# zhoujoey/ORB-SLAM3-Mac

Measured on AMD Instinct MI355X. Metric: ORB extract+match frames/sec, higher is better.
Workload: dtype u8; 1 GPU; vga: synthetic 640x480 batch=1024 per GPU, 8-level pyramid, 1000 feats/frame, ORB extract + Hamming 2-NN match (Frame.cc:1146) + SearchForInitialization (ORBmatcher.cc:710) vs successor frame; pipelines=1, matchers=side by side (two contexts), frames_total=1024

## Files before the change

include/orbhip.h:

```cpp
#ifndef ORBHIP_H
#define ORBHIP_H
#include <stddef.h>
#include <stdint.h>
#ifdef __cplusplus
extern "C" {
#endif

#define ORBHIP_OK 0
#define ORBHIP_E_BADARG (-1)
#define ORBHIP_E_NODEVICE (-2)
#define ORBHIP_E_HIP (-3)
#define ORBHIP_E_CAPACITY (-4)
#define ORBHIP_E_ABORTED (-5)
#define ORBHIP_E_NOTSPD (-6)
#define ORBHIP_E_EMPTY (-7)

typedef struct {
    float x, y, size, angle, response;
    int32_t octave, class_id;
} orbhip_keypoint;

typedef struct orbhip_ctx orbhip_ctx;
typedef struct orbhip_extractor orbhip_extractor;

const char *orbhip_version(void);
const char *orbhip_last_error(void);

int orbhip_ctx_create(int device, void *stream, orbhip_ctx **out);
void orbhip_ctx_destroy(orbhip_ctx *ctx);
int orbhip_ctx_synchronize(orbhip_ctx *ctx);
int orbhip_ctx_wait_for(orbhip_ctx *ctx, orbhip_ctx *other);
int orbhip_ctx_check_status(orbhip_ctx *ctx);
void *orbhip_ctx_stream(orbhip_ctx *ctx);

int orbhip_extractor_create(orbhip_ctx *ctx, int nfeatures, float scale_factor, int nlevels,
                            int ini_th_fast, int min_th_fast, orbhip_extractor **out);
void orbhip_extractor_destroy(orbhip_extractor *ext);

int orbhip_extractor_levels(const orbhip_extractor *ext);
int orbhip_extractor_table(const orbhip_extractor *ext, int which, float *out);
int orbhip_extractor_features_per_level(const orbhip_extractor *ext, int *out);
int orbhip_extractor_umax(const orbhip_extractor *ext, int *out16);

int orbhip_extractor_reserve(orbhip_extractor *ext, int width, int height, int max_batch);
int orbhip_extractor_max_keypoints(const orbhip_extractor *ext);

int orbhip_extract_batch_device(orbhip_extractor *ext, const uint8_t *d_images, int width,
                                int height, size_t row_stride, size_t frame_stride, int batch,
                                int lap0, int lap1);
int orbhip_extractor_results(orbhip_extractor *ext, orbhip_keypoint **d_kp, uint8_t **d_desc,
                             int32_t **d_count, int32_t **d_mono_index);
int orbhip_extract_batch_host(orbhip_extractor *ext, const uint8_t *h_images, int width, int height,
                              size_t row_stride, size_t frame_stride, int batch, int lap0, int lap1,
                              orbhip_keypoint *kp_out, uint8_t *desc_out, int cap,
                              int32_t *count_out, int32_t *mono_out);
int orbhip_extract_batch_host_view(orbhip_extractor *ext, const uint8_t *h_images, int width, int height, size_t row_stride,
                                   size_t frame_stride, int batch, int lap0, int lap1, const orbhip_keypoint **kp_view,
                                   const uint8_t **desc_view, int *row_capacity, const int32_t **count_view, const int32_t **mono_view);
int orbhip_extractor_blur_kernel(const orbhip_extractor *ext, int batch);

int orbhip_extractor_resize_band_rows(const orbhip_extractor *ext, int level);

int orbhip_extractor_last_frame(orbhip_extractor *ext, int frame, const orbhip_keypoint **d_kp, const uint8_t **d_desc,
                                const orbhip_keypoint **h_kp_view, const uint8_t **h_desc_view, int32_t *count, unsigned long long *generation);

int orbhip_extractor_level_dims(const orbhip_extractor *ext, int level, int *w, int *h);
int orbhip_extractor_get_pyramid_level(orbhip_extractor *ext, int frame, int level, int padded,
                                       uint8_t *h_out, size_t out_stride);
int orbhip_extractor_get_pyramid_padded(orbhip_extractor *ext, int frame, uint8_t *const *levels_out, const size_t *strides);
int orbhip_extractor_get_blurred_level(orbhip_extractor *ext, int frame, int level,
                                       uint8_t *h_out, size_t out_stride);
int orbhip_extractor_get_fast_candidates(orbhip_extractor *ext, int frame, int level,
                                         int32_t *xs, int32_t *ys, int32_t *scores, int cap,
                                         int32_t *n_out);
int orbhip_extractor_get_level_keypoints(orbhip_extractor *ext, int frame, int level,
                                         orbhip_keypoint *out, int cap, int32_t *n_out);

int orbhip_extractor_set_graph_mode(orbhip_extractor *ext, int enable);

#define ORBHIP_STAGE_PYRAMID 0
#define ORBHIP_STAGE_FAST_CELLS 1
#define ORBHIP_STAGE_BLUR 2
#define ORBHIP_STAGE_OCTREE 3
#define ORBHIP_STAGE_DESC 4
#define ORBHIP_STAGE_ASSEMBLE 5
#define ORBHIP_STAGE_COUNT 6
int orbhip_extractor_set_profiling(orbhip_extractor *ext, int enable);
int orbhip_extractor_stage_ms(orbhip_extractor *ext, float *ms_out );

int orbhip_descriptor_distance(const uint8_t *a32, const uint8_t *b32);

int orbhip_match_bf2nn_device(orbhip_ctx *ctx, const uint8_t *d_descA, const int32_t *d_nA,
                              size_t strideA, const uint8_t *d_descB, const int32_t *d_nB,
                              size_t strideB, int pairs, int max_n, double ratio,
                              int32_t *d_idx2, int32_t *d_dist2, uint8_t *d_accept);

int orbhip_search_for_initialization_device(orbhip_ctx *ctx,
        const orbhip_keypoint *d_kpA, const uint8_t *d_descA, const int32_t *d_nA,
        const orbhip_keypoint *d_kpB, const uint8_t *d_descB, const int32_t *d_nB,
        int pairs, int max_n, size_t frame_stride_kp , float min_x, float min_y,
        float max_x, float max_y, int window_size, float nn_ratio, int check_orientation,
        float *d_prev_matched, int32_t *d_matches12, int32_t *d_nmatches);

int orbhip_prev_matched_init_device(orbhip_ctx *ctx, const orbhip_keypoint *d_kp, size_t frame_stride_kp,
                                    int frames, int max_n, float *d_prev_matched);

typedef struct orbhip_proj_query {
    float u, v, radius, ur, angle;
    int32_t min_level, max_level, has_obs;
} orbhip_proj_query;
int orbhip_search_by_projection_device(orbhip_ctx *ctx, const orbhip_proj_query *d_q, const uint8_t *d_desc_q,
                                       const int32_t *d_nq, int max_q, const orbhip_keypoint *d_kp,
                                       const uint8_t *d_desc, const float *d_u_right, const int32_t *d_n, int max_n,
                                       size_t frame_stride_kp, int pairs, float min_x, float min_y, float max_x,
                                       float max_y, int th_high, int check_orientation, int32_t *d_train_match,
                                       int32_t *d_nmatches);

int orbhip_search_local_map_device(orbhip_ctx *ctx, const orbhip_proj_query *d_q, const uint8_t *d_desc_q,
                                   const int32_t *d_nq, int max_q, const orbhip_keypoint *d_kp,
                                   const uint8_t *d_desc, const float *d_u_right, const int32_t *d_n, int max_n,
                                   size_t frame_stride_kp, int pairs, float min_x, float min_y, float max_x,
                                   float max_y, int th_high, float nn_ratio, int32_t *d_train_match,
                                   int32_t *d_nmatches);

int orbhip_search_by_projection_rig_device(orbhip_ctx *ctx, int mode, const orbhip_proj_query *d_q, const uint8_t *d_desc_q,
                                           const int32_t *d_nq, int max_q, const orbhip_keypoint *d_kp, const uint8_t *d_desc,
                                           const int32_t *d_n, const int32_t *d_nleft, const int32_t *d_mirror, int max_n,
                                           size_t frame_stride_kp, int pairs, float min_x, float min_y, float max_x, float max_y,
                                           int th_high, float nn_ratio, int check_orientation, int32_t *d_train_match,
                                           int32_t *d_nmatches);

int orbhip_search_by_projection_host(orbhip_ctx *ctx, int mode, const orbhip_proj_query *q, const uint8_t *desc_q, int nq,
                                     const orbhip_keypoint *kp, const uint8_t *desc, const float *u_right, int n,
                                     float min_x, float min_y, float max_x, float max_y, int th_high, float nn_ratio,
                                     int check_orientation, int32_t *train_match_inout, int32_t *nmatches_out);
int orbhip_search_by_projection_rig_host(orbhip_ctx *ctx, int mode, const orbhip_proj_query *q, const uint8_t *desc_q, int nq,
                                         const orbhip_keypoint *kp, const uint8_t *desc, int n, int nleft, const int32_t *mirror,
                                         float min_x, float min_y, float max_x, float max_y, int th_high, float nn_ratio,
                                         int check_orientation, int32_t *train_match_inout, int32_t *nmatches_out);
int orbhip_search_for_initialization_host(orbhip_ctx *ctx, const orbhip_keypoint *kpA, const uint8_t *descA, int nA,
                                          const orbhip_keypoint *kpB, const uint8_t *descB, int nB, float min_x, float min_y,
                                          float max_x, float max_y, int window_size, float nn_ratio, int check_orientation,
                                          float *prev_matched_inout, int32_t *matches12_out, int32_t *nmatches_out);
int orbhip_search_by_projection_host_resident(orbhip_ctx *ctx, int mode, const orbhip_proj_query *q, const uint8_t *desc_q, int nq,
                                              const orbhip_keypoint *kp_host, const orbhip_keypoint *d_kp, const uint8_t *d_desc, const float *u_right, int n,
                                              float min_x, float min_y, float max_x, float max_y, int th_high, float nn_ratio,
                                              int check_orientation, int32_t *train_match_inout, int32_t *nmatches_out);
int orbhip_search_for_initialization_host_resident(orbhip_ctx *ctx, const orbhip_keypoint *kpA, const uint8_t *descA, int nA,
                                                   const orbhip_keypoint *kpB_host, const orbhip_keypoint *d_kpB, const uint8_t *d_descB, int nB, float min_x, float min_y,
                                                   float max_x, float max_y, int window_size, float nn_ratio, int check_orientation,
                                                   float *prev_matched_inout, int32_t *matches12_out, int32_t *nmatches_out);

int orbhip_fuse_search_device(orbhip_ctx *ctx, const orbhip_proj_query *d_q, const uint8_t *d_desc_q, const int32_t *d_nq,
                              int max_q, const orbhip_keypoint *d_kp, const uint8_t *d_desc, const float *d_u_right,
                              const int32_t *d_n, int max_n, size_t frame_stride_kp, int pairs,
                              const float *inv_level_sigma2, int nlevels, float min_x, float min_y, float max_x, float max_y,
                              int32_t *d_best_idx, int32_t *d_best_dist);

int orbhip_search_by_bow_device(orbhip_ctx *ctx,
        const int32_t *d_kf_node_ids, const int32_t *d_kf_node_start, const int32_t *d_kf_feat, const int32_t *d_kf_nnodes,
        const uint8_t *d_kf_valid, const orbhip_keypoint *d_kf_kp, const uint8_t *d_kf_desc,
        const int32_t *d_f_node_ids, const int32_t *d_f_node_start, const int32_t *d_f_feat, const int32_t *d_f_nnodes,
        const orbhip_keypoint *d_f_kp, const uint8_t *d_f_desc, const int32_t *d_nF,
        int pairs, int max_nodes, int max_n, size_t frame_stride_kp, float nn_ratio, int check_orientation,
        int32_t *d_match_f, int32_t *d_nmatches);

int orbhip_search_by_bow_rig_device(orbhip_ctx *ctx,
        const int32_t *d_kf_node_ids, const int32_t *d_kf_node_start, const int32_t *d_kf_feat, const int32_t *d_kf_nnodes,
        const uint8_t *d_kf_valid, const orbhip_keypoint *d_kf_kp, const uint8_t *d_kf_desc,
        const int32_t *d_f_node_ids, const int32_t *d_f_node_start, const int32_t *d_f_feat, const int32_t *d_f_nnodes,
        const orbhip_keypoint *d_f_kp, const uint8_t *d_f_desc, const int32_t *d_nF, const int32_t *d_nleft,
        int pairs, int max_nodes, int max_n, size_t frame_stride_kp, float nn_ratio, int check_orientation,
        int32_t *d_match_f, int32_t *d_nmatches);

int orbhip_search_by_bow_host(orbhip_ctx *ctx,
        const int32_t *kf_node_ids, const int32_t *kf_node_start, const int32_t *kf_feat, int kf_nnodes, const uint8_t *kf_valid,
        const orbhip_keypoint *kf_kp, const uint8_t *kf_desc, int nK,
        const int32_t *f_node_ids, const int32_t *f_node_start, const int32_t *f_feat, int f_nnodes,
        const orbhip_keypoint *f_kp, const uint8_t *f_desc, int nF, int nleft,
        float nn_ratio, int check_orientation, int32_t *match_f_out, int32_t *nmatches_out);
int orbhip_search_by_bow_host_resident(orbhip_ctx *ctx,
        const int32_t *kf_node_ids, const int32_t *kf_node_start, const int32_t *kf_feat, int kf_nnodes, const uint8_t *kf_valid,
        const orbhip_keypoint *kf_kp, const uint8_t *kf_desc, int nK,
        const int32_t *f_node_ids, const int32_t *f_node_start, const int32_t *f_feat, int f_nnodes,
        const orbhip_keypoint *f_kp_host, const orbhip_keypoint *d_f_kp, const uint8_t *d_f_desc, int nF,
        float nn_ratio, int check_orientation, int32_t *match_f_out, int32_t *nmatches_out);

int orbhip_search_by_bow_kf_device(orbhip_ctx *ctx,
        const int32_t *d_node_ids1, const int32_t *d_node_start1, const int32_t *d_feat1, const int32_t *d_nnodes1,
        const uint8_t *d_valid1, const orbhip_keypoint *d_kp1, const uint8_t *d_desc1, const int32_t *d_n1,
        const int32_t *d_node_ids2, const int32_t *d_node_start2, const int32_t *d_feat2, const int32_t *d_nnodes2,
        const uint8_t *d_valid2, const orbhip_keypoint *d_kp2, const uint8_t *d_desc2, const int32_t *d_n2,
        int pairs, int max_nodes, int max_n, size_t frame_stride_kp, float nn_ratio, int check_orientation,
        int32_t *d_matches12, int32_t *d_nmatches);

typedef struct orbhip_tri_pair { float F12[9]; float ep_x, ep_y; int32_t only_stereo, coarse; } orbhip_tri_pair;

int orbhip_search_for_triangulation_device(orbhip_ctx *ctx,
        const int32_t *d_nid1, const uint8_t *d_has_mp1, const orbhip_keypoint *d_kp1, const uint8_t *d_desc1, const float *d_u_right1,
        const int32_t *d_n1,
        const int32_t *d_node_ids2, const int32_t *d_node_start2, const int32_t *d_feat2, const int32_t *d_nnodes2,
        const uint8_t *d_has_mp2, const orbhip_keypoint *d_kp2, const uint8_t *d_desc2, const float *d_u_right2, const int32_t *d_n2,
        const orbhip_tri_pair *d_pair, int pairs, int max_nodes, int max_n, size_t frame_stride_kp,
        const float *scale_factors, const float *level_sigma2, int nlevels, int check_orientation,
        int32_t *d_matches12, int32_t *d_nmatches);

typedef struct orbhip_tri_pair_general {
    float R12[4][9], t12[4][3];
    float F12[4][9];
    float cam1[2][8], cam2[2][8];
    int32_t cam1_type[2], cam2_type[2];
    float ep_x, ep_y;
    int32_t nleft1, nleft2;
    int32_t only_stereo, coarse;
// ... 289 lines not shown
```

orb-slam3-mac_amd/csrc/orb_internal.h:

```cpp
#pragma once
#include <hip/hip_runtime.h>
#include <stdint.h>
#include "../../include/orbhip.h"

#define ORB_MAX_LEVELS 16
#define ORB_EDGE 19
#define ORB_MINB 16
#define ORB_HALF_PATCH 15
#define ORB_RS_STEPS 24

struct OrbLevel {
    uint8_t *img;
    uint8_t *blur;
    size_t img_frame_stride;
    size_t blur_frame_stride;
    int w, h, img_pitch, blur_pitch;
    int ncols, nrows, wcell, hcell;
    int cell_base;
    int cell_cap;
    int quota;
    int key_base, key_cap;
    int kp_base, kp_cap;
    int n_ini;
    float hx;
    float scale;
    float size;
    const int16_t *xofs; const int16_t *xalpha; const int16_t *yofs; const int16_t *ybeta;
    const uint32_t *xchunk; const uint32_t *ytab;
    int resize_mode;
    int rs_rows;
};

struct OrbParams {
    OrbLevel lv[ORB_MAX_LEVELS];
    int nlevels, batch;
    int n_cus;
    int ini_th, min_th;
    int cells_per_frame;
    int keys_per_frame;
    int kps_per_frame;
    int max_kp;
    int oct_nc;
    int rows_min_batch;
    int bm_min_batch;
    int br_blocks[ORB_MAX_LEVELS + 1];
    int bs_tiles[ORB_MAX_LEVELS + 1];
    int lap0, lap1;
    uint32_t *cell_count;
    uint32_t *cell_list;
    size_t cell_list_frame_stride;
    uint32_t *keys;
    uint16_t *node_of;
    uint32_t *lvl_kp;
#define ORB_PERM_MIN_BATCH 16
    uint16_t *lvl_perm;
    float *lvl_angle;
    uint8_t *lvl_desc;
    int32_t *lvl_count;
    int32_t *lvl_ncand;
    int32_t *status;
    orbhip_keypoint *out_kp;
    uint8_t *out_desc;
    int32_t *out_count;
    int32_t *out_mono;
    int umax[ORB_HALF_PATCH + 1];
    int gauss_q8[7];
    const uint4 *bm_th;
    const uint4 *bm_tv;
    int bm_cols[ORB_MAX_LEVELS + 1];
    int bm_init;
};

struct FcLevel {
    const uint8_t *img; size_t frame_stride; int img_pitch;
    int max_bx, max_by;
    int ncols, nrows, wcell, hcell, cell_base, cell_cap;
    int tpr, rpt;
    int rpc, rpr, run_base;
};
struct FastParams {
    FcLevel lv[ORB_MAX_LEVELS];
    int nlevels, batch, ini_th, min_th, cells_per_frame;
    int n_cus;
    int chunk;
    int lvl_lo, lvl_hi;
    uint32_t *cell_count, *cell_list; size_t cell_list_frame_stride; int32_t *status;
    int rows, srows, qcap, wave_dw, small_cells;
    uint32_t div_magic[34];
    int runs_per_frame, run_rows, run_q0, run_dw, use_runs;
};

#define ORB_PACK_KEY(x, y, s) ((uint32_t)(x) | ((uint32_t)(y) << 12) | ((uint32_t)(s) << 24))
#define ORB_KEY_X(k) ((int)((k) & 0xFFFu))
#define ORB_KEY_Y(k) ((int)(((k) >> 12) & 0xFFFu))
#define ORB_KEY_S(k) ((int)((k) >> 24))

struct StereoLevel {
    const uint8_t *imgL, *imgR;
    size_t fsL, fsR;
    int pitchL, pitchR, wR, pad_;
    float scale, inv_scale;
};
struct StereoArgs {
    StereoLevel lv[ORB_MAX_LEVELS];
    int nlevels, batch, max_kp, rows0;
    const orbhip_keypoint *kpL, *kpR;
    const uint8_t *descL, *descR;
    const int32_t *nL, *nR;
    float mb, mbf;
    float *u_right, *depth;
    int32_t *sad, *n_kept;
};
void orb_launch_stereo(const StereoArgs &A, hipStream_t s);

int orb_lds_optin(const void *func, int device, size_t need);

void orb_launch_resize(const OrbParams &P, int level, hipStream_t s);
void orb_launch_fast_cells(const FastParams &F, hipStream_t s, int max_per_cu, int lvl_lo = 0, int lvl_hi = -1);
const void *orb_fast_runs_func(int nld);
#define ORB_OVERLAP_MIN_BATCH 16
#ifndef BLR_R
#define BLR_R 24
#endif
void orb_launch_blur(const OrbParams &P, hipStream_t s, int wgs_per_cu, int frame0 = 0, int nframes = -1);
const void *orb_fast_cells_func(int small);
void orb_launch_octree(const OrbParams &P, hipStream_t s);
void orb_launch_orient_desc(const OrbParams &P, hipStream_t s);
void orb_launch_assemble(const OrbParams &P, hipStream_t s);
size_t orb_octree_lds_bytes(int nc);
int orb_octree_nc(const OrbParams &P);
const void *orb_octree_func();
```

orb-slam3-mac_amd/csrc/orb_kernels.hip:

```cpp
#include "orb_internal.h"
#include "wave_dpp.h"
#include <mutex>
#include <vector>
#include <cstdio>
#include <cstdlib>

#define WAVE 64

__device__ __forceinline__ int wave_incl_scan(int v) { return wave_scan_add_dpp(v); }

__device__ __forceinline__ int block_excl_scan256(int v, int *wsum, int *total)
{
    const int lane = threadIdx.x & (WAVE - 1), wid = threadIdx.x >> 6;
    int inc = wave_incl_scan(v);
    if (lane == WAVE - 1) wsum[wid] = inc;
    __syncthreads();
    int base = 0;
#pragma unroll
    for (int w = 0; w < 4; w++) {
        int s = wsum[w];
        if (w < wid) base += s;
    }
    *total = wsum[0] + wsum[1] + wsum[2] + wsum[3];
    __syncthreads();
// ... 621 lines not shown
#pragma unroll
                for (int i = 0; i < 6; i++) { rm[i] = col[i * PITCH]; rc[i] = col[i * PITCH + 1]; rp[i] = col[i * PITCH + 2]; }
                const uint32_t SIGN = 0x80008000u;
                for (int y0 = 0; y0 < hh; y0 += 7) {
                    const uint32_t *cy = col + y0 * PITCH;
                    uint32_t cm2[7], cp2[7];
#pragma unroll
                    for (int i = 0; i < 7; i++) {
                        rm[6 + i] = cy[(6 + i) * PITCH]; rc[6 + i] = cy[(6 + i) * PITCH + 1]; rp[6 + i] = cy[(6 + i) * PITCH + 2];
                        cm2[i] = cy[(3 + i) * PITCH - 1]; cp2[i] = cy[(3 + i) * PITCH + 3];
                    }
                    bool f[7];
#pragma unroll
                    for (int i = 0; i < 7; i++) {
                        const s16x2 v = as_s16x2(rc[i + 3]);
                        const s16x2 n = as_s16x2(rc[i + 6]), so = as_s16x2(rc[i]);
                        const s16x2 e = pair_odd(cp2[i], rp[i + 3]), w = pair_odd(rm[i + 3], cm2[i]);
                        const s16x2 se = as_s16x2(rp[i + 5]), nw = as_s16x2(rm[i + 1]);
                        const s16x2 ne = as_s16x2(rp[i + 1]), sw = as_s16x2(rm[i + 5]);
                        const s16x2 lo = pkmax(pkmax3(pkmin(n, so), pkmin(e, w), pkmin(se, nw)), pkmin(ne, sw));
                        const s16x2 hi = pkmin(pkmin3(pkmax(n, so), pkmax(e, w), pkmax(se, nw)), pkmax(ne, sw));
                        const s16x2 M = pkmax(v - lo, hi - v);
                        f[i] = y0 + i < rows_on && (as_u32(M - thP) & SIGN) != SIGN;
                    }
#pragma unroll
                    for (int i = 0; i < 7; i++) {
                        const unsigned long long b = __ballot(f[i]);
                        const uint32_t blo = (uint32_t)b, bhi = (uint32_t)(b >> 32);
                        const int m = (int)__builtin_amdgcn_mbcnt_hi(bhi, __builtin_amdgcn_mbcnt_lo(blo, 0u));
                        const int pos = m + (half ? q0cap + nq1 - __popc(blo) : nq0);
                        if (f[i]) Q[pos] = (uint16_t)FC_ID(rb + y0 + i, bp);
                        nq0 += __popc(blo); nq1 += __popc(bhi);
                    }
#pragma unroll
                    for (int i = 0; i < 6; i++) { rm[i] = rm[7 + i]; rc[i] = rc[7 + i]; rp[i] = rp[7 + i]; }
                }
            }
            const int nq = nq0 + nq1;
            FC_WAVE_SYNC();
            for (int i0 = 0; i0 < nq; i0 += 64) {
                const int i = min(i0 + lane, nq - 1);
                const int id = Q[i < nq0 ? i : q0cap + i - nq0], by = id >> 5, qp = id & 31;
                const s16x2 S = fc_arc_score<PITCH>(&PT[(by + 3) * PITCH + qp + 2]);
                if (i0 + lane < nq) {
                    const uint32_t lo = S.x > lo_th ? (uint32_t)(S.x - 1) : 0u;
                    const uint32_t hi = (S.y > lo_th && 2 * qp + 1 < dw) ? (uint32_t)(S.y - 1) : 0u;
                    SC[(by + 1) * SPITCH + qp + 1] = (uint16_t)(lo | (hi << 8));
                }
            }
            FC_WAVE_SYNC();
            for (int i0 = 0; i0 < nq; i0 += 64) {
                const int i = i0 + lane;
                uint32_t keep = 0, sc = 0;
                int by = 0, qp = 0;
                if (i < nq) {
                    const int id = Q[i < nq0 ? i : q0cap + i - nq0];
                    by = id >> 5; qp = id & 31;
                    const uint16_t *q = &SC[(by + 1) * SPITCH + qp + 1];
#define FC_U(v) as_s16x2(__builtin_amdgcn_perm(0u, (uint32_t)(v), 0x0c010c00u))
                    sc = q[0];
                    const s16x2 V = pkmax(FC_U(q[-SPITCH]), FC_U(q[SPITCH]));
                    const s16x2 Lc = pkmax3(FC_U(q[-SPITCH - 1]), FC_U(q[-1]), FC_U(q[SPITCH - 1]));
                    const s16x2 Rc = pkmax3(FC_U(q[-SPITCH + 1]), FC_U(q[1]), FC_U(q[SPITCH + 1]));
#undef FC_U
                    const int xl = 2 * qp, xr = xl + 1;
                    const int sl = (int)(sc & 0xFFu), sr = (int)(sc >> 8);
                    const int nbl = max(max((int)V.x, xl != B ? (int)Lc.y : 0), xr != B ? max((int)V.y, sr) : 0);
                    const int nbr = max(max((int)V.y, xr + 1 != B ? (int)Rc.x : 0), xr != B ? max((int)V.x, sl) : 0);
                    const bool onL = !pass || ((xl >= B ? 2u : 1u) & empty), onR = !pass || ((xr >= B ? 2u : 1u) & empty);
                    if (sl >= th && sl > nbl && onL) keep |= 1u;
                    if (sr >= th && sr > nbr && onR) keep |= 2u;
                }
                const int xl = 2 * qp;
                const bool kL = keep & 1u, kR = keep & 2u, cL = xl >= B, cR = xl + 1 >= B;
#pragma unroll
                for (int c = 0; c < 2; c++) {
                    const bool mL = kL && (int)cL == c, mR = kR && (int)cR == c;
                    const unsigned long long bL = __ballot(mL), bR = __ballot(mR);
                    const int before = (int)__builtin_amdgcn_mbcnt_hi((uint32_t)(bL >> 32), __builtin_amdgcn_mbcnt_lo((uint32_t)bL, 0u)) +
                                       (int)__builtin_amdgcn_mbcnt_hi((uint32_t)(bR >> 32), __builtin_amdgcn_mbcnt_lo((uint32_t)bR, 0u));
                    const int base = c ? tot1 : tot0;
                    uint32_t *lst = list + (size_t)c * cell_cap;
                    if (mL) { const int o = base + before; if (o < cell_cap) lst[o] = ORB_PACK_KEY(xl + key_x0, by + key_y0, sc & 0xFFu); }
                    if (mR) { const int o = base + before + (mL ? 1 : 0); if (o < cell_cap) lst[o] = ORB_PACK_KEY(xl + 1 + key_x0, by + key_y0, (sc >> 8) & 0xFFu); }
                    const int add = __popcll(bL) + __popcll(bR);
                    if (c) tot1 += add; else tot0 += add;
                }
            }
            if (pass || min_th == ini_th) break;
            empty = (tot0 == 0 && dw0 > 0 ? 1u : 0u) | (tot1 == 0 && dw1 > 0 ? 2u : 0u);
            if (!empty) break;
            FC_WAVE_SYNC();
        }
        if (tot0 > cell_cap || tot1 > cell_cap) { if (lane == 0) atomicExch(P.status, ORBHIP_E_CAPACITY); tot0 = min(tot0, cell_cap); tot1 = min(tot1, cell_cap); }
        if (lane == 0) { cnt_out[0] = (uint32_t)tot0; if (nc > 1) cnt_out[1] = (uint32_t)tot1; }
        C = N;
    }
#undef FC_WAVE_SYNC
}
const void *orb_fast_runs_func(int nld) { return nld == 4 ? reinterpret_cast<const void *>(k_fast_runs<4>) : reinterpret_cast<const void *>(k_fast_runs<6>); }

const void *orb_fast_cells_func(int small);
void orb_launch_fast_cells(const FastParams &F_, hipStream_t s, int max_per_cu, int lvl_lo, int lvl_hi)
{
    FastParams F = F_;
    F.lvl_lo = lvl_lo; F.lvl_hi = lvl_hi < 0 ? F.nlevels : lvl_hi;
    if (F.lvl_lo >= F.lvl_hi) return;
    const bool runs = F.use_runs != 0;
    const size_t lds = sizeof(uint32_t) * (size_t)(runs ? F.run_dw : F.wave_dw);
    const int nld = (F.run_rows - 7) * FR_NCH <= 256 ? 4 : 6;
    const int v = runs ? (nld == 4 ? 2 : 3) : F.small_cells ? 1 : 0;
    int per_cu;
    {
        struct Occ { int dev, v, n; size_t lds; };
        static std::mutex occ_mu; static std::vector<Occ> occ_tab;
        int dev = 0; (void)hipGetDevice(&dev);
        std::lock_guard<std::mutex> g(occ_mu);
        const Occ *hit = nullptr;
        for (const Occ &o : occ_tab) if (o.dev == dev && o.v == v && o.lds == lds) { hit = &o; break; }
        if (!hit) {
            int n = 0;
            if (hipOccupancyMaxActiveBlocksPerMultiprocessor(&n, v >= 2 ? orb_fast_runs_func(nld) : orb_fast_cells_func(v), 64, lds) != hipSuccess || n < 1) n = (int)((160 * 1024) / (lds + 512));
            occ_tab.push_back(Occ{dev, v, n < 1 ? 1 : n, lds}); hit = &occ_tab.back();
            if (getenv("ORBHIP_DEBUG_FAST")) fprintf(stderr, "[orbhip] %s: %zu B of LDS per wave, %d waves per CU resident\n", v >= 2 ? "k_fast_runs" : "k_fast_cells", lds, hit->n);
        }
        per_cu = hit->n;
    }
    if (max_per_cu > 0 && per_cu > max_per_cu) per_cu = max_per_cu;
    long nblocks = (long)(F.n_cus > 0 ? F.n_cus : 256) * per_cu;
    const long total = runs ? (long)F.batch * ((F.lvl_hi < F.nlevels ? F.lv[F.lvl_hi].run_base : F.runs_per_frame) - F.lv[F.lvl_lo].run_base)
                            : (long)F.batch * ((F.lvl_hi < F.nlevels ? F.lv[F.lvl_hi].cell_base : F.cells_per_frame) - F.lv[F.lvl_lo].cell_base);
    if (nblocks > total) nblocks = (total + 7) / 8 * 8;
    static const int chunk_env = getenv("ORBHIP_TUNE_FAST_CHUNK") ? atoi(getenv("ORBHIP_TUNE_FAST_CHUNK")) : 0;
    const long fair = total / (8 * nblocks);
    const int cmax = runs ? 8 : 4;
    F.chunk = chunk_env > 0 ? chunk_env : (int)(fair < 1 ? 1 : fair > cmax ? cmax : fair);
    if (runs && nld == 4) hipLaunchKernelGGL(k_fast_runs<4>, dim3((unsigned)nblocks), dim3(64), lds, s, F);
    else if (runs) hipLaunchKernelGGL(k_fast_runs<6>, dim3((unsigned)nblocks), dim3(64), lds, s, F);
    else if (F.small_cells) hipLaunchKernelGGL((k_fast_cells<3, 24, 2>), dim3((unsigned)nblocks), dim3(64), lds, s, F);
    else hipLaunchKernelGGL((k_fast_cells<5, 32, 5>), dim3((unsigned)nblocks), dim3(64), lds, s, F);
}
const void *orb_fast_cells_func(int small) { return small ? reinterpret_cast<const void *>(k_fast_cells<3, 24, 2>) : reinterpret_cast<const void *>(k_fast_cells<5, 32, 5>); }

struct OctLds {
    uint32_t *cc;
    int *ord;
    int *by_ord;
    int *excl;
    int *posbase;
    int *newpos;
    uint32_t *best;
};

int orb_octree_nc(const OrbParams &P)
{
    int nc = 0;
    for (int l = 0; l < P.nlevels; l++) { const int a = P.lv[l].quota + 16, b = 4 * P.lv[l].n_ini + 4; nc = a > nc ? a : nc; nc = b > nc ? b : nc; }
    return nc;
}

size_t orb_octree_lds_bytes(int nc)
{
    return (size_t)nc * 4 * (6 + 4 + 6) + 64;
}

__device__ __forceinline__ int oct_quadrant(uint32_t key, uint32_t b0, uint32_t b1)
{
    const int x0 = b0 & 0xFFFF, y0 = b0 >> 16, x1 = b1 & 0xFFFF, y1 = b1 >> 16;
    const int mx = x0 + ((x1 - x0 + 1) >> 1), my = y0 + ((y1 - y0 + 1) >> 1);
    const int kx = ORB_KEY_X(key), ky = ORB_KEY_Y(key);
    return (kx < mx ? 0 : 1) + (ky < my ? 0 : 2);
}

#define OCT_KR 8
#ifdef OCT_PROF
__device__ long long g_oct_prof[8];
#define OCT_T(i) do { if (blockIdx.x == 0 && threadIdx.x == 0) { const long long t_ = clock64(); g_oct_prof[i] += t_ - t_prev; t_prev = t_; } } while (0)
extern "C" int orbhip_debug_oct_prof(long long *out8, int reset)
{
    if (out8 && hipMemcpyFromSymbol(out8, HIP_SYMBOL(g_oct_prof), 64) != hipSuccess) return -1;
    if (reset) { long long z[8] = {0}; if (hipMemcpyToSymbol(HIP_SYMBOL(g_oct_prof), z, 64) != hipSuccess) return -1; }
    return 0;
}
#else
#define OCT_T(i) do { } while (0)
#endif
__global__ __launch_bounds__(256) void k_octree(OrbParams P)
{
    extern __shared__ uint32_t smem[];
    __shared__ int wsum[8];
    __shared__ int s_size, s_front, s_nexpand, s_rstar, s_T, s_nproc;
    const int tid = threadIdx.x;
#ifdef OCT_PROF
    long long t_prev = clock64();
#endif
    const int lvl = blockIdx.x / P.batch;
    const int frame = blockIdx.x - lvl * P.batch;
    const OrbLevel &L = P.lv[lvl];
    const int N = L.quota;
    const int NC = P.oct_nc;
    uint32_t *box0 = smem, *box1 = smem + NC, *cnt = smem + 2 * NC;
    uint32_t *nbox0 = smem + 3 * NC, *nbox1 = smem + 4 * NC, *ncnt = smem + 5 * NC;
    OctLds S;
    {
        uint32_t *p = smem + 6 * NC;
        S.cc = p; p += 4 * NC;
        S.ord = (int *)p; p += NC; S.by_ord = (int *)p; p += NC; S.excl = (int *)p; p += NC;
        S.posbase = (int *)p; p += NC; S.newpos = (int *)p; p += NC; S.best = p; p += NC;
    }
    const uint32_t *ccount = P.cell_count + (size_t)frame * P.cells_per_frame + L.cell_base;
    const uint32_t *clist = P.cell_list + (size_t)frame * P.cell_list_frame_stride + (size_t)L.cell_base * L.cell_cap;
    uint32_t *keys = P.keys + (size_t)frame * P.keys_per_frame + L.key_base;
    uint16_t *node_of = P.node_of + (size_t)frame * P.keys_per_frame + L.key_base;
    const int ncells = L.ncols * L.nrows;
    uint32_t rk[OCT_KR]; int rn[OCT_KR];
    int running = 0;
    int32_t *count_out = P.lvl_count + frame * P.nlevels + lvl;
    if (ncells + 1 <= 16 * NC) {
        int *coff = reinterpret_cast<int *>(smem);
        for (int c0 = 0; c0 < ncells; c0 += 256) {
            const int c = c0 + tid;
            const int n = c < ncells ? min((int)ccount[c], L.cell_cap) : 0;
            int total;
            const int off = running + block_excl_scan256(n, wsum, &total);
            if (c < ncells) coff[c] = off;
            running += total;
        }
        if (tid == 0) coff[ncells] = running;
        __syncthreads();
        if (running > L.key_cap) { if (tid == 0) atomicExch(P.status, ORBHIP_E_CAPACITY); running = L.key_cap; }
        const int K0 = running;
        auto fetch = [&](int k) {
            int lo = 0, hi = ncells;
            while (hi - lo > 1) { const int mid = (lo + hi) >> 1; if (coff[mid] <= k) lo = mid; else hi = mid; }
            return clist[(size_t)lo * L.cell_cap + (k - coff[lo])];
        };
#pragma unroll
        for (int i = 0; i < OCT_KR; i++) { const int k = tid + 256 * i; rk[i] = k < K0 ? fetch(k) : 0u; rn[i] = 0; }
#pragma unroll
        for (int i = 0; i < OCT_KR; i++) { const int k = tid + 256 * i; if (k < K0) keys[k] = rk[i]; }
        for (int k = tid + 256 * OCT_KR; k < K0; k += 256) keys[k] = fetch(k);
        __syncthreads();
    } else {
        for (int c0 = 0; c0 < ncells; c0 += 256) {
            const int c = c0 + tid;
            const int n = c < ncells ? (int)ccount[c] : 0;
            int total;
            const int off = running + block_excl_scan256(n, wsum, &total);
            for (int i = 0; i < n; i++)
                if (off + i < L.key_cap) keys[off + i] = clist[(size_t)c * L.cell_cap + i];
            running += total;
        }
        if (running > L.key_cap) { if (tid == 0) atomicExch(P.status, ORBHIP_E_CAPACITY); running = L.key_cap; }
        __syncthreads();
        __threadfence_block();
#pragma unroll
        for (int i = 0; i < OCT_KR; i++) { const int k = tid + 256 * i; rk[i] = k < running ? keys[k] : 0u; rn[i] = 0; }
    }
    const int K = running;
    if (tid == 0) P.lvl_ncand[frame * P.nlevels + lvl] = K;
    if (K == 0) { if (tid == 0) *count_out = 0; return; }
    __syncthreads();
    __threadfence_block();
    OCT_T(0);
    const int n_ini = L.n_ini;
    const int H = (L.h - ORB_MINB) - ORB_MINB;
    for (int i = tid; i < NC; i += 256) { cnt[i] = 0; ncnt[i] = 0; }
    __syncthreads();
#pragma unroll
    for (int i = 0; i < OCT_KR; i++)
        if (tid + 256 * i < K) {
            const int r = (int)__fdiv_rn((float)ORB_KEY_X(rk[i]), L.hx);
            rn[i] = r;
            atomicAdd(&ncnt[r], 1u);
        }
    for (int k = tid + 256 * OCT_KR; k < K; k += 256) {
        const int r = (int)__fdiv_rn((float)ORB_KEY_X(keys[k]), L.hx);
        node_of[k] = (uint16_t)r;
        atomicAdd(&ncnt[r], 1u);
    }
    __syncthreads();
    if (tid == 0) {
        int m = 0;
        for (int i = 0; i < n_ini; i++) {
            const uint32_t c = ncnt[i];
            S.newpos[i] = m;
            if (c) {
                box0[m] = (uint32_t)(int)__fmul_rn(L.hx, (float)i);
                box1[m] = (uint32_t)(int)__fmul_rn(L.hx, (float)(i + 1)) | ((uint32_t)H << 16);
                cnt[m] = c;
                m++;
            }
        }
        s_size = m; s_front = m;
    }
    __syncthreads();
#pragma unroll
    for (int i = 0; i < OCT_KR; i++) if (tid + 256 * i < K) rn[i] = S.newpos[rn[i]];
    for (int k = tid + 256 * OCT_KR; k < K; k += 256) node_of[k] = (uint16_t)S.newpos[node_of[k]];
    __syncthreads();

    OCT_T(1);
    bool final_phase = false;
    int size = s_size, front = s_front;
    for (int guard = 0; guard < 64; guard++) {
        int C;
        if (!final_phase) {
            int run = 0;
            for (int p0 = 0; p0 < size; p0 += 256) {
                const int p = p0 + tid;
                const int f = (p < size && cnt[p] > 1) ? 1 : 0;
                int tot;
                const int o = run + block_excl_scan256(f, wsum, &tot);
                if (p < size) { S.ord[p] = f ? o : -1; if (f) S.by_ord[o] = p; }
                run += tot;
            }
            C = run;
        } else {
            int run = 0;
            for (int p0 = 0; p0 < size; p0 += 256) {
                const int p = p0 + tid;
                const int f = (p < front && cnt[p] > 1) ? 1 : 0;
                int tot;
                const int o = run + block_excl_scan256(f, wsum, &tot);
                if (p < size) S.ord[p] = -1;
                if (f) S.excl[o] = p;
                run += tot;
            }
            C = run;
            __syncthreads();
            for (int i = tid; i < C; i += 256) {
                const int p = S.excl[i];
                const uint32_t ci = cnt[p];
                int r = 0;
                for (int j = 0; j < C; j++) {
                    const uint32_t cj = cnt[S.excl[j]];
                    r += (cj > ci || (cj == ci && j < i)) ? 1 : 0;
                }
                S.ord[p] = r;
                S.by_ord[r] = p;
            }
        }
        __syncthreads();
        if (C == 0) break;
        for (int i = tid; i < 4 * size; i += 256) S.cc[i] = 0;
        if (tid == 0) { s_nexpand = 0; s_rstar = C - 1; }
        __syncthreads();
#pragma unroll
        for (int i = 0; i < OCT_KR; i++)
            if (tid + 256 * i < K) {
                const int p = rn[i];
                if (S.ord[p] >= 0) atomicAdd(&S.cc[4 * p + oct_quadrant(rk[i], box0[p], box1[p])], 1u);
            }
        for (int k = tid + 256 * OCT_KR; k < K; k += 256) {
            const int p = node_of[k];
            if (S.ord[p] >= 0) atomicAdd(&S.cc[4 * p + oct_quadrant(keys[k], box0[p], box1[p])], 1u);
        }
        __syncthreads();
        {
            int run = 0;
            for (int o0 = 0; o0 < C; o0 += 256) {
                const int o = o0 + tid;
                int nch = 0;
                if (o < C) { const uint32_t *q = &S.cc[4 * S.by_ord[o]]; nch = (q[0] > 0) + (q[1] > 0) + (q[2] > 0) + (q[3] > 0); }
                int tot;
                const int e = run + block_excl_scan256(nch, wsum, &tot);
                if (o < C) {
                    S.excl[o] = e;
                    if (final_phase && size + e + nch - (o + 1) >= N) atomicMin(&s_rstar, o);
                }
                run += tot;
            }
        }
        __syncthreads();
        const int rstar = s_rstar;
        int T, nproc;
        {
            const uint32_t *q = &S.cc[4 * S.by_ord[rstar]];
            T = S.excl[rstar] + (q[0] > 0) + (q[1] > 0) + (q[2] > 0) + (q[3] > 0);
            nproc = rstar + 1;
        }
        {
            int run = 0;
            for (int p0 = 0; p0 < size; p0 += 256) {
                const int p = p0 + tid;
                const int surv = (p < size && !(S.ord[p] >= 0 && S.ord[p] <= rstar)) ? 1 : 0;
                int tot;
                const int e = run + block_excl_scan256(surv, wsum, &tot);
                if (p < size && surv) S.newpos[p] = T + e;
                run += tot;
            }
        }
        for (int p = tid; p < size; p += 256) {
            const int o = S.ord[p];
            if (o >= 0 && o <= rstar) {
                const uint32_t *q = &S.cc[4 * p];
                const int nch = (q[0] > 0) + (q[1] > 0) + (q[2] > 0) + (q[3] > 0);
                const int base = T - (S.excl[o] + nch);
                S.posbase[p] = base;
                const uint32_t b0 = box0[p], b1 = box1[p];
                const int x0 = b0 & 0xFFFF, y0 = b0 >> 16, x1 = b1 & 0xFFFF, y1 = b1 >> 16;
                const int mx = x0 + ((x1 - x0 + 1) >> 1), my = y0 + ((y1 - y0 + 1) >> 1);
                int pos = base, nexp = 0;
                for (int qd = 3; qd >= 0; qd--) {
                    if (q[qd]) {
                        const int cx0 = (qd & 1) ? mx : x0, cx1 = (qd & 1) ? x1 : mx;
                        const int cy0 = (qd & 2) ? my : y0, cy1 = (qd & 2) ? y1 : my;
                        nbox0[pos] = (uint32_t)cx0 | ((uint32_t)cy0 << 16);
                        nbox1[pos] = (uint32_t)cx1 | ((uint32_t)cy1 << 16);
                        ncnt[pos] = q[qd];
                        nexp += q[qd] > 1;
                        pos++;
                    }
                }
                if (nexp) atomicAdd(&s_nexpand, nexp);
            } else {
                const int np = S.newpos[p];
                nbox0[np] = box0[p]; nbox1[np] = box1[p]; ncnt[np] = cnt[p];
            }
        }
        __syncthreads();
        auto relabel = [&](uint32_t key, int p) {
            const int o = S.ord[p];
            if (o >= 0 && o <= rstar) {
                const int qd = oct_quadrant(key, box0[p], box1[p]);
                const uint32_t *q = &S.cc[4 * p];
                int r = 0;
                for (int j = 3; j > qd; j--) r += q[j] > 0;
                return S.posbase[p] + r;
            }
            return S.newpos[p];
        };
#pragma unroll
        for (int i = 0; i < OCT_KR; i++) if (tid + 256 * i < K) rn[i] = relabel(rk[i], rn[i]);
        for (int k = tid + 256 * OCT_KR; k < K; k += 256) node_of[k] = (uint16_t)relabel(keys[k], node_of[k]);
        __syncthreads();
        const int new_size = T + (size - nproc);
        const int nexpand = s_nexpand;
        { uint32_t *t; t = box0; box0 = nbox0; nbox0 = t; t = box1; box1 = nbox1; nbox1 = t; t = cnt; cnt = ncnt; ncnt = t; }
        const int old_size = size;
        size = new_size; front = T;
#ifdef OCT_PROF
        if (blockIdx.x == 0 && tid == 0) g_oct_prof[5] += 1;
#endif
        if (new_size >= N || new_size == old_size) break;
        if (!final_phase && new_size + 3 * nexpand > N) final_phase = true;
    }
    __syncthreads();
    OCT_T(2);
    for (int i = tid; i < size; i += 256) S.best[i] = 0;
    __syncthreads();
#pragma unroll
    for (int i = 0; i < OCT_KR; i++)
        if (tid + 256 * i < K) atomicMax(&S.best[rn[i]], ((uint32_t)ORB_KEY_S(rk[i]) << 20) | (uint32_t)(0xFFFFF - (tid + 256 * i)));
    for (int k = tid + 256 * OCT_KR; k < K; k += 256)
        atomicMax(&S.best[node_of[k]], ((uint32_t)ORB_KEY_S(keys[k]) << 20) | (uint32_t)(0xFFFFF - k));
    __syncthreads();
    OCT_T(3);
    uint32_t *out = P.lvl_kp + (size_t)frame * P.kps_per_frame + L.kp_base;
    int nout = size;
    if (nout > L.kp_cap) { if (tid == 0) atomicExch(P.status, ORBHIP_E_CAPACITY); nout = L.kp_cap; }
    uint16_t *perm = P.lvl_perm + (size_t)frame * P.kps_per_frame + L.kp_base;
    for (int i = tid; i < nout; i += 256) out[i] = keys[0xFFFFF - (S.best[i] & 0xFFFFF)];
    if (P.batch < ORB_PERM_MIN_BATCH) { if (tid == 0) *count_out = nout; return; }
    __syncthreads();
    for (int i = tid; i < nout; i += 256) { const uint32_t ki = out[i]; S.best[i] = ((uint32_t)(ORB_KEY_Y(ki) >> 5) << 16) | (uint32_t)ORB_KEY_X(ki); }
    __syncthreads();
    for (int i = tid; i < nout; i += 256) {
        const uint32_t si = S.best[i];
        int rank = 0;
        for (int j = 0; j < nout; j++) { const uint32_t sj = S.best[j]; rank += (sj < si) || (sj == si && j < i); }
        perm[rank] = (uint16_t)i;
    }
    if (tid == 0) *count_out = nout;
    OCT_T(4);
}

const void *orb_octree_func() { return reinterpret_cast<const void *>(k_octree); }

void orb_launch_octree(const OrbParams &P, hipStream_t s)
{
    const size_t lds = orb_octree_lds_bytes(P.oct_nc);
    hipLaunchKernelGGL(k_octree, dim3(P.nlevels * P.batch), dim3(256), lds, s, P);
}

#define BL_TW 64
#define BL_TH 32
#define BL_ROWS (BL_TH + 6)
#define BL_IPD 20
__device__ __forceinline__ int reflect101(int p, int n)
{
    if (p < 0) p = -p;
    if (p >= n) p = 2 * n - 2 - p;
    return p;
}

__device__ __forceinline__ uint32_t bl_load4(const uint8_t *row, int x, int w)
{
    if (x >= 0 && x + 3 < w) return *reinterpret_cast<const uint32_t *>(row + x);
    uint32_t v = 0;
#pragma unroll
    for (int j = 0; j < 4; j++) {
        int xx = reflect101(x + j, w);
        xx = min(max(xx, 0), w - 1);
        v |= (uint32_t)row[xx] << (8 * j);
    }
    return v;
}

__device__ __forceinline__ void bl_row4(uint32_t d0, uint32_t d1, uint32_t d2, uint32_t klo, uint32_t khi, uint32_t (&o)[4])
{
    o[0] = __builtin_amdgcn_udot4(__builtin_amdgcn_alignbyte(d1, d0, 1), klo, __builtin_amdgcn_udot4(__builtin_amdgcn_alignbyte(d2, d1, 1), khi, 0u, false), false);
    o[1] = __builtin_amdgcn_udot4(__builtin_amdgcn_alignbyte(d1, d0, 2), klo, __builtin_amdgcn_udot4(__builtin_amdgcn_alignbyte(d2, d1, 2), khi, 0u, false), false);
    o[2] = __builtin_amdgcn_udot4(__builtin_amdgcn_alignbyte(d1, d0, 3), klo, __builtin_amdgcn_udot4(__builtin_amdgcn_alignbyte(d2, d1, 3), khi, 0u, false), false);
    o[3] = __builtin_amdgcn_udot4(d1, klo, __builtin_amdgcn_udot4(d2, khi, 0u, false), false);
}

typedef unsigned short u16x2 __attribute__((ext_vector_type(2)));
__device__ __forceinline__ uint32_t bl_dot2(uint32_t a, uint32_t b, uint32_t c)
{
    return __builtin_amdgcn_udot2(__builtin_bit_cast(u16x2, a), __builtin_bit_cast(u16x2, b), c, false);
}

struct BlTile { int level, frame, tx, ty, ntx, nty, w, h, pitch; const uint8_t *src; uint8_t *dst; int dpitch; };
__device__ __forceinline__ void bl_tile_level(const OrbParams &P, BlTile &T)
{
    const OrbLevel &L = P.lv[T.level];
    T.w = __builtin_amdgcn_readfirstlane(L.w); T.h = __builtin_amdgcn_readfirstlane(L.h);
    T.pitch = __builtin_amdgcn_readfirstlane(L.img_pitch); T.dpitch = __builtin_amdgcn_readfirstlane(L.blur_pitch);
    T.ntx = (T.w + BL_TW - 1) / BL_TW; T.nty = (T.h + BL_TH - 1) / BL_TH;
}
__device__ __forceinline__ void bl_tile_frame(const OrbParams &P, BlTile &T)
{
    const OrbLevel &L = P.lv[T.level];
    T.src = L.img + (size_t)T.frame * L.img_frame_stride; T.dst = L.blur + (size_t)T.frame * L.blur_frame_stride;
}
__device__ __forceinline__ uint4 bl_stage_load(const BlTile &T, int tid)
{
    const bool chunk = tid < 4 * BL_ROWS;
    const int a = tid - 4 * BL_ROWS;
    const int r = chunk ? tid >> 2 : a >> 1;
    const int x0 = T.tx * BL_TW, y0 = T.ty * BL_TH, w = T.w;
    int y = reflect101(y0 + r - 3, T.h);
    y = min(max(y, 0), T.h - 1);
    const uint8_t *row = T.src + (uint32_t)__umul24((uint32_t)y, (uint32_t)T.pitch);
    uint4 v = make_uint4(0, 0, 0, 0);
    if (chunk) {
        const int x = x0 + 16 * (tid & 3);
        if (x + 15 < w) v = *reinterpret_cast<const uint4 *>(row + x);
        else { v.x = bl_load4(row, x, w); v.y = bl_load4(row, x + 4, w); v.z = bl_load4(row, x + 8, w); v.w = bl_load4(row, x + 12, w); }
    } else if (a < 2 * BL_ROWS) {
        v.x = bl_load4(row, (a & 1) ? x0 + BL_TW : x0 - 4, w);
    }
    return v;
}

__global__ __launch_bounds__(256) void k_blur(OrbParams P)
{
    __shared__ __attribute__((aligned(16))) uint32_t in[BL_ROWS * BL_IPD + 4];
    __shared__ __attribute__((aligned(16))) uint32_t hz2[(BL_ROWS / 2) * BL_TW];
    const int tid = threadIdx.x;
    const unsigned lid = xcd_logical_id(blockIdx.x, gridDim.x);
    const long total = (long)P.bs_tiles[P.nlevels] * P.batch;
    const long t0 = total * lid / gridDim.x, t1 = total * (lid + 1) / gridDim.x;
    if (t0 >= t1) return;
    BlTile T;
    {
        T.level = 0;
        for (int l = 1; l < P.nlevels; l++) if (t0 >= (long)P.bs_tiles[l] * P.batch) T.level = l;
        bl_tile_level(P, T);
        const long rel = t0 - (long)P.bs_tiles[T.level] * P.batch;
        T.frame = (int)(rel / (T.ntx * T.nty));
        const int trem = (int)(rel - (long)T.frame * (T.ntx * T.nty));
        T.ty = trem / T.ntx; T.tx = trem - T.ty * T.ntx;
        bl_tile_frame(P, T);
    }
    const uint32_t klo = (uint32_t)P.gauss_q8[0] | ((uint32_t)P.gauss_q8[1] << 8) | ((uint32_t)P.gauss_q8[2] << 16) | ((uint32_t)P.gauss_q8[3] << 24);
    const uint32_t khi = (uint32_t)P.gauss_q8[4] | ((uint32_t)P.gauss_q8[5] << 8) | ((uint32_t)P.gauss_q8[6] << 16);
    const uint32_t k0 = P.gauss_q8[0], k1 = P.gauss_q8[1], k2 = P.gauss_q8[2], k3 = P.gauss_q8[3];
    const uint32_t wt[2][4] = {{k0 | (k1 << 16), k2 | (k3 << 16), k2 | (k1 << 16), k0},
                               {k0 << 16, k1 | (k2 << 16), k3 | (k2 << 16), k1 | (k0 << 16)}};
    const bool chunk = tid < 4 * BL_ROWS;
    const int sa = tid - 4 * BL_ROWS;
    const int sidx = chunk ? (tid >> 2) * BL_IPD + 4 + 4 * (tid & 3) : (sa >> 1) * BL_IPD + ((sa & 1) ? BL_IPD : 3);
    auto advance = [&](BlTile &X) {
        X.tx++;
        if (X.tx == X.ntx) { X.tx = 0; X.ty++; }
        if (X.ty == X.nty) {
            X.ty = 0; X.frame++;
            if (X.frame == P.batch) { X.frame = 0; X.level++; bl_tile_level(P, X); }
            bl_tile_frame(P, X);
        }
    };
    auto body = [&](uint4 &ld, BlTile &T, long t) {
        const int x0 = T.tx * BL_TW, y0 = T.ty * BL_TH, w = T.w, h = T.h, dpitch = T.dpitch;
        uint8_t *bdst = T.dst;
        if (chunk) *reinterpret_cast<uint4 *>(&in[sidx]) = ld;
        else if (sa < 2 * BL_ROWS) in[sidx] = ld.x;
        __syncthreads();
        if (t + 1 < t1) { advance(T); ld = bl_stage_load(T, tid); }
        for (int i = tid; i < (BL_ROWS / 2) * (BL_TW / 4); i += 256) {
            const int rp = i >> 4, c4 = i & 15;
            const uint32_t *q = &in[2 * rp * BL_IPD + 3 + c4];
            uint32_t oa[4], ob[4];
            bl_row4(q[0], q[1], q[2], klo, khi, oa);
            bl_row4(q[BL_IPD], q[BL_IPD + 1], q[BL_IPD + 2], klo, khi, ob);
            uint4 pk;
            pk.x = oa[0] | (ob[0] << 16); pk.y = oa[1] | (ob[1] << 16); pk.z = oa[2] | (ob[2] << 16); pk.w = oa[3] | (ob[3] << 16);
            *reinterpret_cast<uint4 *>(&hz2[rp * BL_TW + 4 * c4]) = pk;
        }
        __syncthreads();
        {
            const int c4 = tid & 15, rg = tid >> 4;
            const int x = x0 + 4 * c4;
            if (x < w) {
                uint4 pr[4];
#pragma unroll
                for (int k = 0; k < 4; k++) pr[k] = *reinterpret_cast<const uint4 *>(&hz2[(rg + k) * BL_TW + 4 * c4]);
#pragma unroll
                for (int rr = 0; rr < 2; rr++) {
                    const int y = y0 + 2 * rg + rr;
                    if (y < h) {
                        uint32_t acc[4];
#pragma unroll
                        for (int j = 0; j < 4; j++) {
                            uint32_t a = 32768u;
#pragma unroll
                            for (int k = 0; k < 4; k++) {
                                const uint32_t pv = j == 0 ? pr[k].x : j == 1 ? pr[k].y : j == 2 ? pr[k].z : pr[k].w;
                                a = bl_dot2(pv, wt[rr][k], a);
                            }
                            acc[j] = min(a, 0x00FFFFFFu);
                        }
                        const uint32_t p01 = __builtin_amdgcn_perm(acc[1], acc[0], 0x0c0c0602u);
                        const uint32_t p23 = __builtin_amdgcn_perm(acc[3], acc[2], 0x0c0c0602u);
                        *reinterpret_cast<uint32_t *>(bdst + (uint32_t)__umul24((uint32_t)y, (uint32_t)dpitch) + x) = p01 | (p23 << 16);
// ... 449 lines not shown
```

orb-slam3-mac_amd/csrc/orbhip_api.hip:

```cpp
#include "orb_internal.h"
#include <cmath>
#include <cfloat>
#include <cstdio>
#include <cstdlib>
#include <cstring>
#include <string>
#include <vector>
#include <mutex>
#include <set>
#include <utility>

static thread_local std::string g_last_error;
extern "C" const char *orbhip_last_error(void) { return g_last_error.c_str(); }
extern "C" const char *orbhip_version(void) { return "orbhip 0.1 (gfx950)"; }

#define HIP_TRY(expr)                                                                   \
    do {                                                                                \
        hipError_t _e = (expr);                                                         \
        if (_e != hipSuccess) {                                                         \
            g_last_error = std::string(#expr) + ": " + hipGetErrorString(_e);           \
            return ORBHIP_E_HIP;                                                        \
        }                                                                               \
    } while (0)

// ... 48 lines not shown
    else {
        hipError_t e2 = hipStreamCreateWithFlags(&c->stream, hipStreamNonBlocking);
        if (e2 != hipSuccess) { delete c; g_last_error = hipGetErrorString(e2); return ORBHIP_E_HIP; }
        c->own_stream = true;
    }
    if (hipMalloc((void **)&c->d_status, sizeof(int32_t)) != hipSuccess || hipMemset(c->d_status, 0, sizeof(int32_t)) != hipSuccess) {
        if (c->own_stream) (void)hipStreamDestroy(c->stream);
        delete c; g_last_error = "hipMalloc(status)"; return ORBHIP_E_HIP;
    }
    c->status_redirect = nullptr;
    c->scratch = nullptr; c->scratch_bytes = 0; c->work = nullptr; c->work_bytes = 0; c->ba_schur_mode = 0; c->n_cus = 0; c->pinned = nullptr; c->pinned_bytes = 0; c->ba_arena = nullptr; c->ba_arena_bytes = 0; c->ba_arena_busy = false; c->pinned_word = nullptr;
    if (hipDeviceGetAttribute(&c->n_cus, hipDeviceAttributeMultiprocessorCount, device) != hipSuccess || c->n_cus <= 0) c->n_cus = 256;
    *out = c;
    return ORBHIP_OK;
}
void *orbhip_ctx_scratch_internal(orbhip_ctx *c, size_t bytes)
{
    if (bytes <= c->scratch_bytes) return c->scratch;
    (void)hipStreamSynchronize(c->stream);
    if (c->scratch) (void)hipFree(c->scratch);
    c->scratch = nullptr; c->scratch_bytes = 0;
    const size_t want = std::max<size_t>(bytes + bytes / 2, 1 << 20);
    if (hipMalloc(&c->scratch, want) != hipSuccess) { g_last_error = "hipMalloc(scratch arena)"; return nullptr; }
    c->scratch_bytes = want;
    return c->scratch;
}
void *orbhip_ctx_pinned_internal(orbhip_ctx *c, size_t bytes)
{
    if (bytes <= c->pinned_bytes) return c->pinned;
    (void)hipStreamSynchronize(c->stream);
    if (c->pinned) (void)hipHostFree(c->pinned);
    c->pinned = nullptr; c->pinned_bytes = 0;
    const size_t want = std::max<size_t>(bytes + bytes / 2, 1 << 20);
    if (hipHostMalloc(&c->pinned, want, hipHostMallocDefault) != hipSuccess) { g_last_error = "hipHostMalloc(pinned staging arena)"; return nullptr; }
    c->pinned_bytes = want;
    return c->pinned;
}
void *orbhip_ctx_ba_arena_acquire_internal(orbhip_ctx *c, size_t bytes)
{
    if (c->ba_arena_busy) return nullptr;
    if (bytes > c->ba_arena_bytes) {
        (void)hipStreamSynchronize(c->stream);
        if (c->ba_arena) (void)hipFree(c->ba_arena);
        c->ba_arena = nullptr; c->ba_arena_bytes = 0;
        const size_t want = bytes + bytes / 4;
        if (hipMalloc(&c->ba_arena, want) != hipSuccess) return nullptr;
        c->ba_arena_bytes = want;
    }
    c->ba_arena_busy = true;
    return c->ba_arena;
}
void orbhip_ctx_ba_arena_release_internal(orbhip_ctx *c) { c->ba_arena_busy = false; }
int *orbhip_ctx_pinned_word_internal(orbhip_ctx *c)
{
    if (!c->pinned_word && hipHostMalloc((void **)&c->pinned_word, 256, hipHostMallocDefault) != hipSuccess) c->pinned_word = nullptr;
    return c->pinned_word;
}
void *orbhip_ctx_work_internal(orbhip_ctx *c, size_t bytes)
{
    if (bytes <= c->work_bytes) return c->work;
    (void)hipStreamSynchronize(c->stream);
    if (c->work) (void)hipFree(c->work);
    c->work = nullptr; c->work_bytes = 0;
    const size_t want = std::max<size_t>(bytes + bytes / 4, 1 << 20);
    if (hipMalloc(&c->work, want) != hipSuccess) { g_last_error = "hipMalloc(work arena)"; return nullptr; }
    c->work_bytes = want;
    return c->work;
}
void orbhip_set_last_error_internal(const char *msg) { g_last_error = msg; }
int32_t *orbhip_ctx_status_internal(orbhip_ctx *c);
extern "C" int orbhip_ctx_check_status(orbhip_ctx *c)
{
    if (!c) return ORBHIP_E_BADARG;
    int32_t st = 0;
    HIP_TRY(hipStreamSynchronize(c->stream));
    HIP_TRY(hipMemcpy(&st, orbhip_ctx_status_internal(c), sizeof(st), hipMemcpyDeviceToHost));
    if (st) { HIP_TRY(hipMemset(orbhip_ctx_status_internal(c), 0, sizeof(int32_t))); g_last_error = "device-side capacity exceeded in a matcher kernel"; }
    return st;
}
int32_t *orbhip_ctx_status_internal(orbhip_ctx *c) { return c->status_redirect ? c->status_redirect : c->d_status; }
void orbhip_ctx_redirect_status_internal(orbhip_ctx *c, int32_t *p) { c->status_redirect = p; }
extern "C" void orbhip_ctx_destroy(orbhip_ctx *c)
{
    if (!c) return;
    (void)hipFree(c->d_status);
    if (c->scratch) (void)hipFree(c->scratch);
    if (c->work) (void)hipFree(c->work);
    if (c->pinned) (void)hipHostFree(c->pinned);
    if (c->ba_arena) (void)hipFree(c->ba_arena);
    if (c->pinned_word) (void)hipHostFree(c->pinned_word);
    if (c->own_stream) (void)hipStreamDestroy(c->stream);
    delete c;
}
extern "C" int orbhip_ctx_synchronize(orbhip_ctx *c)
{
    if (!c) return ORBHIP_E_BADARG;
    HIP_TRY(hipStreamSynchronize(c->stream));
    return ORBHIP_OK;
}
extern "C" int orbhip_ctx_wait_for(orbhip_ctx *c, orbhip_ctx *other)
{
    if (!c || !other) return ORBHIP_E_BADARG;
    if (c == other || c->stream == other->stream) return ORBHIP_OK;
    if (c->device != other->device) { g_last_error = "orbhip_ctx_wait_for: contexts of two devices"; return ORBHIP_E_BADARG; }
    HIP_TRY(hipSetDevice(c->device));
    hipEvent_t ev;
    HIP_TRY(hipEventCreateWithFlags(&ev, hipEventDisableTiming));
    HIP_TRY(hipEventRecord(ev, other->stream));
    HIP_TRY(hipStreamWaitEvent(c->stream, ev, 0));
    HIP_TRY(hipEventDestroy(ev));
    return ORBHIP_OK;
}
extern "C" void *orbhip_ctx_stream(orbhip_ctx *c) { return c ? (void *)c->stream : nullptr; }
hipStream_t orbhip_ctx_stream_internal(orbhip_ctx *c) { return c->stream; }
int orbhip_ctx_device_internal(orbhip_ctx *c) { return c->device; }
int orbhip_ctx_cus_internal(orbhip_ctx *c) { return c->n_cus; }
int orbhip_ctx_ba_schur_mode_internal(orbhip_ctx *c) { return c->ba_schur_mode; }
extern "C" int orbhip_ctx_set_ba_schur_mode(orbhip_ctx *c, int mode)
{
    if (!c || mode < 0 || mode > 2) return ORBHIP_E_BADARG;
    c->ba_schur_mode = mode;
    return ORBHIP_OK;
}

static inline int cv_round_f(float v) { return (int)lrintf(v); }
static inline int cv_round_d(double v) { return (int)lrint(v); }
static inline int align_up(int v, int a) { return (v + a - 1) / a * a; }

#define ORBHIP_PROF_SLOTS 32
struct orbhip_extractor {
    orbhip_ctx *ctx;
    int nfeatures, nlevels, ini_th, min_th;
    float scale_factor;
    float scale[ORB_MAX_LEVELS], inv_scale[ORB_MAX_LEVELS], sigma2[ORB_MAX_LEVELS], inv_sigma2[ORB_MAX_LEVELS];
    int per_level[ORB_MAX_LEVELS];
    int umax[ORB_HALF_PATCH + 1];
    int gauss_q8[7];
    int width, height, max_batch;
    bool level0_owned;
    OrbParams P;
    FastParams F;
    std::vector<void *> allocs;
    size_t bytes_reserved;
    int last_batch;
    bool profiling;
    hipEvent_t ev[ORBHIP_PROF_SLOTS][ORBHIP_STAGE_COUNT + 1];
    int ev_calls;
    bool ev_created;
    float stage_ms[ORBHIP_STAGE_COUNT];
    uint8_t *d_level0;
    int32_t *d_stereo_sad;
    bool graph_mode, graph_valid;
    hipStream_t aux; hipEvent_t ev_fork, ev_join, ev_pyr; bool aux_ok; int overlap;
    hipGraphExec_t graph_exec;
    int g_w, g_h, g_batch, g_lap0, g_lap1;
    size_t level0_frame_stride; int level0_pitch;
    uint8_t *d_outblob; size_t outblob_bytes, ob_kp, ob_desc;
    uint8_t *h_out; uint8_t *h_in; size_t h_in_bytes; int32_t *h_status;
    uint8_t *h_pyr; size_t h_pyr_bytes;
    unsigned long long generation, view_generation;
};

extern "C" int orbhip_extractor_create(orbhip_ctx *ctx, int nfeatures, float scale_factor, int nlevels,
                                       int ini_th, int min_th, orbhip_extractor **out)
{
    if (!ctx || !out || nlevels < 1 || nlevels > ORB_MAX_LEVELS || nfeatures < 1 || !(scale_factor > 1.0f) || scale_factor > 2.0f)
        return ORBHIP_E_BADARG;
    orbhip_extractor *e = new orbhip_extractor();
    e->ctx = ctx; e->nfeatures = nfeatures; e->nlevels = nlevels; e->ini_th = ini_th; e->min_th = min_th;
    e->scale_factor = scale_factor;
    e->width = e->height = e->max_batch = 0; e->bytes_reserved = 0; e->last_batch = 0;
    e->profiling = false; e->ev_created = false; e->ev_calls = 0; e->d_level0 = nullptr; e->level0_owned = false;
    e->d_stereo_sad = nullptr;
    e->graph_mode = false; e->graph_valid = false; e->graph_exec = nullptr;
    e->aux = nullptr; e->ev_fork = e->ev_join = e->ev_pyr = nullptr; e->aux_ok = false; e->overlap = 1;
    e->d_outblob = nullptr; e->outblob_bytes = e->ob_kp = e->ob_desc = 0; e->h_out = e->h_in = e->h_pyr = nullptr; e->h_in_bytes = e->h_pyr_bytes = 0; e->h_status = nullptr;
    e->generation = 0; e->view_generation = ~0ull;
    memset(&e->P, 0, sizeof(e->P));
    memset(e->stage_ms, 0, sizeof(e->stage_ms));
    e->scale[0] = 1.0f; e->sigma2[0] = 1.0f;
    for (int i = 1; i < nlevels; i++) { e->scale[i] = e->scale[i - 1] * scale_factor; e->sigma2[i] = e->scale[i] * e->scale[i]; }
    for (int i = 0; i < nlevels; i++) { e->inv_scale[i] = 1.0f / e->scale[i]; e->inv_sigma2[i] = 1.0f / e->sigma2[i]; }
    float factor = 1.0f / scale_factor;
    float desired = nfeatures * (1 - factor) / (1 - (float)pow((double)factor, (double)nlevels));
    int sum = 0;
    for (int l = 0; l < nlevels - 1; l++) { e->per_level[l] = cv_round_f(desired); sum += e->per_level[l]; desired *= factor; }
    e->per_level[nlevels - 1] = std::max(nfeatures - sum, 0);
    int v, v0, vmax = (int)floor(ORB_HALF_PATCH * sqrtf(2.f) / 2 + 1), vmin = (int)ceil(ORB_HALF_PATCH * sqrtf(2.f) / 2);
    const double hp2 = ORB_HALF_PATCH * ORB_HALF_PATCH;
    for (v = 0; v <= vmax; ++v) e->umax[v] = cv_round_d(sqrt(hp2 - v * v));
    for (v = ORB_HALF_PATCH, v0 = 0; v >= vmin; --v) { while (e->umax[v0] == e->umax[v0 + 1]) ++v0; e->umax[v] = v0; ++v0; }
    {
        float cf[7]; double s = 0;
        for (int i = 0; i < 7; i++) { double x = i - 3.0; cf[i] = (float)exp(-0.5 / 4.0 * x * x); s += cf[i]; }
        s = 1. / s;
        for (int i = 0; i < 7; i++) { cf[i] = (float)(cf[i] * s); e->gauss_q8[i] = cv_round_f(cf[i] * 256.f); }
    }
    *out = e;
    return ORBHIP_OK;
}

static void ext_free_all(orbhip_extractor *e)
{
    for (void *p : e->allocs) (void)hipFree(p);
    e->allocs.clear();
    e->bytes_reserved = 0; e->width = e->height = e->max_batch = 0; e->d_level0 = nullptr; e->d_stereo_sad = nullptr;
    if (e->h_out) (void)hipHostFree(e->h_out);
    if (e->h_in) (void)hipHostFree(e->h_in);
    if (e->h_pyr) (void)hipHostFree(e->h_pyr);
    if (e->h_status) (void)hipHostFree(e->h_status);
    e->h_out = e->h_in = e->h_pyr = nullptr; e->h_status = nullptr; e->h_in_bytes = e->h_pyr_bytes = 0; e->d_outblob = nullptr; e->view_generation = ~0ull;
    if (e->graph_valid) { (void)hipGraphExecDestroy(e->graph_exec); e->graph_valid = false; }
}
static void ext_free_aux(orbhip_extractor *e)
{
    if (!e->aux_ok) return;
    (void)hipStreamSynchronize(e->aux);
    (void)hipEventDestroy(e->ev_fork); (void)hipEventDestroy(e->ev_join); (void)hipEventDestroy(e->ev_pyr); (void)hipStreamDestroy(e->aux);
    e->aux_ok = false;
}

extern "C" void orbhip_extractor_destroy(orbhip_extractor *e)
{
    if (!e) return;
    (void)hipStreamSynchronize(e->ctx->stream);
    ext_free_aux(e);
    ext_free_all(e);
    if (e->ev_created) for (auto &slot : e->ev) for (auto &ev : slot) (void)hipEventDestroy(ev);
    delete e;
}

extern "C" int orbhip_extractor_levels(const orbhip_extractor *e) { return e ? e->nlevels : ORBHIP_E_BADARG; }
extern "C" int orbhip_extractor_table(const orbhip_extractor *e, int which, float *out)
{
    if (!e || !out || which < 0 || which > 3) return ORBHIP_E_BADARG;
    const float *t = which == 0 ? e->scale : which == 1 ? e->inv_scale : which == 2 ? e->sigma2 : e->inv_sigma2;
    memcpy(out, t, sizeof(float) * e->nlevels);
    return ORBHIP_OK;
}
extern "C" int orbhip_extractor_features_per_level(const orbhip_extractor *e, int *out)
{
    if (!e || !out) return ORBHIP_E_BADARG;
    memcpy(out, e->per_level, sizeof(int) * e->nlevels);
    return ORBHIP_OK;
}
extern "C" int orbhip_extractor_umax(const orbhip_extractor *e, int *out16)
{
    if (!e || !out16) return ORBHIP_E_BADARG;
    memcpy(out16, e->umax, sizeof(int) * 16);
    return ORBHIP_OK;
}
extern "C" int orbhip_extractor_max_keypoints(const orbhip_extractor *e) { return e ? e->P.max_kp : ORBHIP_E_BADARG; }

template <typename T>
static int dev_alloc(orbhip_extractor *e, T **p, size_t count)
{
    void *q = nullptr;
    size_t bytes = std::max<size_t>(count * sizeof(T), 256);
    hipError_t err = hipMalloc(&q, bytes);
    if (err != hipSuccess) { g_last_error = std::string("hipMalloc: ") + hipGetErrorString(err); return ORBHIP_E_HIP; }
    e->allocs.push_back(q);
    e->bytes_reserved += bytes;
    *p = (T *)q;
    return ORBHIP_OK;
}

static void resize_tables(int sn, int dn, bool horizontal, std::vector<int16_t> &ofs, std::vector<int16_t> &coef)
{
    double scale = 1. / ((double)dn / sn);
    ofs.resize(dn); coef.resize(2 * dn);
    for (int d = 0; d < dn; d++) {
        float f = (float)((d + 0.5) * scale - 0.5);
        int s = (int)floorf(f);
        f -= s;
        if (horizontal) {
            if (s < 0) { f = 0; s = 0; }
            if (s >= sn - 1) { f = 0; s = sn - 1; }
        }
        int c0 = cv_round_f((1.f - f) * 2048), c1 = cv_round_f(f * 2048);
        ofs[d] = (int16_t)std::min(std::max(s, -32768), 32767);
        coef[2 * d] = (int16_t)std::min(std::max(c0, -32768), 32767);
        coef[2 * d + 1] = (int16_t)std::min(std::max(c1, -32768), 32767);
    }
}

extern "C" int orbhip_extractor_reserve(orbhip_extractor *e, int width, int height, int max_batch)
{
    if (!e || width <= 0 || height <= 0 || max_batch <= 0) return ORBHIP_E_BADARG;
    if (e->width == width && e->height == height && e->max_batch >= max_batch) return ORBHIP_OK;
    if (width > 4096 + 2 * ORB_MINB || height > 4096 + 2 * ORB_MINB) { g_last_error = "image larger than 12-bit key packing"; return ORBHIP_E_BADARG; }
    HIP_TRY(hipSetDevice(e->ctx->device));
    HIP_TRY(hipStreamSynchronize(e->ctx->stream));
    ext_free_all(e);
    OrbParams &P = e->P;
    memset(&P, 0, sizeof(P));
    P.nlevels = e->nlevels; P.ini_th = e->ini_th; P.min_th = e->min_th;
    memcpy(P.umax, e->umax, sizeof(P.umax));
    memcpy(P.gauss_q8, e->gauss_q8, sizeof(P.gauss_q8));
    int cells = 0, keys = 0, kps = 0, max_cell_cap = 0;
    for (int l = 0; l < e->nlevels; l++) {
        OrbLevel &L = P.lv[l];
        L.w = cv_round_f((float)width * e->inv_scale[l]);
        L.h = cv_round_f((float)height * e->inv_scale[l]);
        const float w_ = (float)((L.w - ORB_EDGE + 3) - ORB_MINB), h_ = (float)((L.h - ORB_EDGE + 3) - ORB_MINB);
        if (w_ < 30.f || h_ < 30.f) { g_last_error = "pyramid level smaller than one FAST cell"; return ORBHIP_E_BADARG; }
        L.ncols = (int)(w_ / 30.f); L.nrows = (int)(h_ / 30.f);
        L.wcell = (int)ceilf(w_ / L.ncols); L.hcell = (int)ceilf(h_ / L.nrows);
        if (L.wcell + 6 > 64 || L.hcell + 6 > 64) { g_last_error = "FAST cell exceeds the 64x64 LDS tile"; return ORBHIP_E_BADARG; }
        max_cell_cap = std::max(max_cell_cap, ((L.wcell + 1) / 2) * ((L.hcell + 1) / 2));
        L.cell_base = cells; cells += L.ncols * L.nrows;
        L.quota = e->per_level[l];
        const int maxx = L.w - ORB_MINB, maxy = L.h - ORB_MINB;
        L.n_ini = (int)roundf((float)(maxx - ORB_MINB) / (maxy - ORB_MINB));
        if (L.n_ini < 1) { g_last_error = "nIni == 0 (image taller than 2x its width): undefined in the reference"; return ORBHIP_E_BADARG; }
        L.hx = (float)(maxx - ORB_MINB) / L.n_ini;
        L.scale = e->scale[l];
        L.size = (float)(int)(31 * e->scale[l]);
        L.kp_base = kps; L.kp_cap = align_up(std::max(L.quota + 8, 4 * L.n_ini + 4), 4); kps += L.kp_cap;
    }
    for (int l = 0; l < e->nlevels; l++) {
        OrbLevel &L = P.lv[l];
        L.cell_cap = max_cell_cap;
        L.key_base = keys;
        L.key_cap = std::min(L.ncols * L.nrows * max_cell_cap, ((L.w - 2 * ORB_MINB + 1) / 2 + L.ncols) * ((L.h - 2 * ORB_MINB + 1) / 2 + L.nrows));
        L.key_cap = std::min(L.key_cap, 0xFFFFF);
        keys += align_up(L.key_cap, 4);
    }
    P.cells_per_frame = cells; P.keys_per_frame = keys; P.kps_per_frame = kps; P.max_kp = align_up(kps, 8);
    {
        FastParams &F = e->F;
        memset(&F, 0, sizeof(F));
        int mw = 0, mh = 0;
        bool small = true;
        for (int l = 0; l < e->nlevels; l++) {
            const OrbLevel &L = P.lv[l];
            FcLevel &f = F.lv[l];
            mw = std::max(mw, L.wcell); mh = std::max(mh, L.hcell);
            f.max_bx = L.w - ORB_MINB; f.max_by = L.h - ORB_MINB;
            f.ncols = L.ncols; f.nrows = L.nrows; f.wcell = L.wcell; f.hcell = L.hcell; f.cell_base = L.cell_base; f.cell_cap = L.cell_cap;
            const int npb = (L.wcell + 1) >> 1, nq = (npb + 5) >> 1;
            f.tpr = (npb + 1) >> 1; f.rpt = 64 / f.tpr;
            (void)nq;
            small = small && npb + 4 <= 24 && npb + 2 <= 24 && (L.hcell + 6) * 3 <= 64 * 2;
        }
        {
            int runs = 0;
            bool ok = true;
            for (int l = 0; l < e->nlevels; l++) {
                const OrbLevel &L = P.lv[l];
                FcLevel &f = F.lv[l];
                f.rpc = 2 * L.wcell <= 64 ? 2 : 1;
                f.rpr = (L.ncols + f.rpc - 1) / f.rpc;
                f.run_base = runs; runs += f.rpr * L.nrows;
                ok = ok && L.wcell <= 64 && L.hcell + 6 <= 70 && L.wcell >= 8 && L.hcell >= 8;
            }
            const int hh = (mh + 1) / 2;
            F.runs_per_frame = runs;
            F.run_rows = mh + 6 + 7;
            F.run_q0 = (hh * 32 + 7) & ~7;
            F.run_dw = F.run_rows * 40 + (((mh + 2) * 40 + 2 * F.run_q0) + 1) / 2;
            F.run_dw = (F.run_dw + 3) & ~3;
            F.use_runs = ok && getenv("ORBHIP_FAST_KERNEL") && !strcmp(getenv("ORBHIP_FAST_KERNEL"), "runs") ? 1 : 0;
        }
        const int npb = (mw + 1) >> 1;
        F.small_cells = small ? 1 : 0;
        F.rows = mh + 6; F.srows = mh; F.qcap = (mh * npb + 1) & ~1;
        F.wave_dw = F.rows * (small ? 24 : 40) + ((F.srows + 2) * (small ? 24 : 32) + F.qcap + 1) / 2;
        F.wave_dw = (F.wave_dw + 3) & ~3;
        F.nlevels = e->nlevels; F.ini_th = e->ini_th; F.min_th = e->min_th; F.cells_per_frame = cells;
        for (int n = 1; n < 34; n++) F.div_magic[n] = (uint32_t)(65536 / n + 1);
    }
    P.bs_tiles[0] = 0;
    for (int l = 0; l < e->nlevels; l++) P.bs_tiles[l + 1] = P.bs_tiles[l] + ((P.lv[l].w + 63) / 64) * ((P.lv[l].h + 31) / 32);
    P.rows_min_batch = getenv("ORBHIP_ROWS_MIN_BATCH") ? atoi(getenv("ORBHIP_ROWS_MIN_BATCH")) : 16;
    {
        bool ok = !getenv("ORBHIP_BLUR_TILES");
        P.br_blocks[0] = 0;
        for (int l = 0; l < e->nlevels; l++) {
            const int w = P.lv[l].w, h = P.lv[l].h;
            if (h < BLR_R + 4 || w < 16) ok = false;
            P.br_blocks[l + 1] = P.br_blocks[l] + (((w + 3) / 4) * ((h + BLR_R - 1) / BLR_R) + 255) / 256;
        }
        if (!ok) P.br_blocks[e->nlevels] = 0;
    }
    P.cell_list_frame_stride = (size_t)cells * max_cell_cap;
    int rc;
    const size_t B = (size_t)max_batch;
    for (int l = 0; l < e->nlevels; l++) {
        OrbLevel &L = P.lv[l];
        L.img_pitch = align_up(L.w, 64); L.blur_pitch = L.img_pitch;
        L.img_frame_stride = (size_t)L.img_pitch * L.h; L.blur_frame_stride = L.img_frame_stride;
        if ((rc = dev_alloc(e, &L.img, B * L.img_frame_stride + 64))) return rc;
        if ((rc = dev_alloc(e, &L.blur, B * L.blur_frame_stride + 64))) return rc;
        if (l > 0) {
            std::vector<int16_t> xo, xa, yo, yb;
            resize_tables(P.lv[l - 1].w, L.w, true, xo, xa);
            resize_tables(P.lv[l - 1].h, L.h, false, yo, yb);
            int16_t *dxo, *dxa, *dyo, *dyb;
            if ((rc = dev_alloc(e, &dxo, xo.size()))) return rc;
            if ((rc = dev_alloc(e, &dxa, xa.size()))) return rc;
            if ((rc = dev_alloc(e, &dyo, yo.size()))) return rc;
            if ((rc = dev_alloc(e, &dyb, yb.size()))) return rc;
            HIP_TRY(hipMemcpy(dxo, xo.data(), xo.size() * 2, hipMemcpyHostToDevice));
            HIP_TRY(hipMemcpy(dxa, xa.data(), xa.size() * 2, hipMemcpyHostToDevice));
            HIP_TRY(hipMemcpy(dyo, yo.data(), yo.size() * 2, hipMemcpyHostToDevice));
            HIP_TRY(hipMemcpy(dyb, yb.data(), yb.size() * 2, hipMemcpyHostToDevice));
            L.xofs = dxo; L.xalpha = dxa; L.yofs = dyo; L.ybeta = dyb;
            const int sw = P.lv[l - 1].w, sh = P.lv[l - 1].h, nch = (L.w + 3) / 4;
            std::vector<uint32_t> xc((size_t)nch * 12, 0), yt;
            bool fits = sw >= 8 && nch >= 4;
            const char *rm = getenv("ORBHIP_RESIZE_MODE");
            int mode = l > 1 || (sw % 4 == 0 && sw >= 12) ? 1 : 0;
            if (rm && atoi(rm) == 0) mode = 0;
            for (int c = 0; c < nch && fits; c++) {
                const int base = std::min((int)xo[4 * c], sw - 8);
                const int base4 = l > 1 ? (base & ~3) : std::min(base & ~3, sw - 12);
                xc[12 * c] = mode ? (uint32_t)base4 : (uint32_t)base;
                xc[12 * c + 9] = 0x03020100u + 0x01010101u * (uint32_t)(base - base4);
                for (int j = 0; j < 4; j++) {
                    const int col = std::min(4 * c + j, L.w - 1);
                    const int i0 = xo[col] - base, a0 = xa[2 * col], a1 = xa[2 * col + 1];
                    int i1 = i0 + 1;
                    if (i0 < 0 || i0 > 7 || a0 < 0 || a1 < 0) { fits = false; break; }
                    if (i1 > 7) { if (a1 != 0) { fits = false; break; } i1 = i0; }
                    xc[12 * c + 1 + j] = (uint32_t)i0 | 0x0c00u | ((uint32_t)i1 << 16) | 0x0c000000u;
                    xc[12 * c + 5 + j] = (uint32_t)a0 | ((uint32_t)a1 << 16);
                }
            }
            for (int dy = 0; dy < L.h; dy++)
                if (yb[2 * dy] < 0 || yb[2 * dy + 1] < 0 || yb[2 * dy] > 2048 || yb[2 * dy + 1] > 2048) fits = false;
            auto band_steps = [&](int y0, int y1, std::vector<uint32_t> *out) {
                int n = 0, prev = -1;
                for (int dy = y0; dy < y1; dy++) {
                    const int r0 = std::min(std::max((int)yo[dy], 0), sh - 1), r1 = std::min(std::max((int)yo[dy] + 1, 0), sh - 1);
                    if (n == 0 || prev != r0) {
                        if (out) { const uint32_t e[4] = {(uint32_t)r0, 0u, 0u, 0u}; out->insert(out->end(), e, e + 4); }
                        n++;
                    }
                    if (out) { const uint32_t e[4] = {(uint32_t)r1, 1u, (uint32_t)yb[2 * dy] << 12, (uint32_t)yb[2 * dy + 1] << 12}; out->insert(out->end(), e, e + 4); }
                    n++; prev = r1;
                }
                return n;
            };
            int rsr = ORB_RS_STEPS - 1;
            for (; rsr > 1; rsr--) {
                bool ok = true;
                for (int y0 = 0; y0 < L.h && ok; y0 += rsr) ok = band_steps(y0, std::min(y0 + rsr, L.h), nullptr) <= ORB_RS_STEPS;
                if (ok) break;
            }
            L.rs_rows = rsr;
            for (int y0 = 0; y0 < L.h && fits; y0 += rsr) {
                const size_t at = yt.size();
                band_steps(y0, std::min(y0 + rsr, L.h), &yt);
                while (yt.size() < at + 4 * ORB_RS_STEPS) {
                    const uint32_t e[4] = {yt[yt.size() - 4], 0u, 0u, 0u};
                    yt.insert(yt.end(), e, e + 4);
                }
            }
            L.xchunk = nullptr; L.ytab = nullptr;
            if (fits && !getenv("ORBHIP_RESIZE_TILES")) {
                uint32_t *dxc, *dyt;
                if ((rc = dev_alloc(e, &dxc, xc.size()))) return rc;
                if ((rc = dev_alloc(e, &dyt, yt.size()))) return rc;
                HIP_TRY(hipMemcpy(dxc, xc.data(), xc.size() * 4, hipMemcpyHostToDevice));
                HIP_TRY(hipMemcpy(dyt, yt.data(), yt.size() * 4, hipMemcpyHostToDevice));
                L.xchunk = dxc; L.ytab = dyt;
                L.resize_mode = mode;
            }
        }
    }
    e->d_level0 = P.lv[0].img; e->level0_pitch = P.lv[0].img_pitch; e->level0_frame_stride = P.lv[0].img_frame_stride;
    {
        const char *bm_env = getenv("ORBHIP_BLUR_MFMA");
        const bool bm_force = bm_env && atoi(bm_env) == 1, bm_off = bm_env && atoi(bm_env) == 0;
        bool ok = !bm_off && (bm_force || (size_t)width * height <= (size_t)320 * 1024) && P.br_blocks[e->nlevels] > 0;
        P.bm_min_batch = bm_force ? P.rows_min_batch : 128;
        int S = 0;
        for (int i = 0; i < 7; i++) { S += e->gauss_q8[i]; if (e->gauss_q8[i] < 0 || e->gauss_q8[i] > 63) ok = false; }
        if (255 * S > 65535) ok = false;
        P.bm_cols[0] = 0;
        for (int l = 0; l < e->nlevels; l++) {
            if (P.lv[l].w < 32 || P.lv[l].h < 8) ok = false;
            P.bm_cols[l + 1] = P.bm_cols[l] + (P.lv[l].w + 31) / 32;
        }
        auto refl = [](int x, int n) { return x < 0 ? -x : (x >= n ? 2 * n - 2 - x : x); };
        std::vector<int8_t> th((size_t)P.bm_cols[e->nlevels] * 2 * 64 * 16, 0), tv((size_t)4 * 64 * 16, 0);
        for (int l = 0; l < e->nlevels && ok; l++) {
            const int w = P.lv[l].w;
            for (int tx = 0; tx < (w + 31) / 32; tx++) {
                int cxs[4];
                for (int g = 0; g < 4; g++) { int cx = 32 * tx - 16 + 16 * g; cx = cx < 0 ? 0 : cx; if (cx + 16 > w) cx = w - 16; cxs[g] = cx; }
                for (int cb = 0; cb < 2; cb++)
                    for (int n = 0; n < 16; n++) {
                        const int xo = 32 * tx + 16 * cb + n;
                        if (xo >= w) continue;
                        for (int i = -3; i <= 3; i++) {
                            const int col = refl(xo + i, w);
                            int gp = -1;
                            for (int g = 0; g < 4 && gp < 0; g++) if (col >= cxs[g] && col < cxs[g] + 16) gp = g;
                            if (gp < 0) { ok = false; break; }
                            int8_t &c = th[((((size_t)(P.bm_cols[l] + tx) * 2 + cb) * 64) + (size_t)(n + 16 * gp)) * 16 + (col - cxs[gp])];
                            c = (int8_t)(c + e->gauss_q8[i + 3]);
                        }
                    }
            }
        }
        for (int b = 0; b < 4; b++)
            for (int lane = 0; lane < 64; lane++)
                for (int j = 0; j < 16; j++) {
                    const int n = lane & 15, g = lane >> 4, krow = 16 * (j >> 2) + 4 * g + (j & 3), d = krow - (16 * b + n);
                    tv[((size_t)b * 64 + lane) * 16 + j] = (int8_t)((d >= 0 && d <= 6) ? e->gauss_q8[d] : 0);
                }
        P.bm_th = nullptr; P.bm_tv = nullptr; P.bm_init = 128 * S;
        if (ok) {
            uint4 *dth, *dtv;
            if ((rc = dev_alloc(e, &dth, th.size() / 16))) return rc;
            if ((rc = dev_alloc(e, &dtv, tv.size() / 16))) return rc;
            HIP_TRY(hipMemcpy(dth, th.data(), th.size(), hipMemcpyHostToDevice));
            HIP_TRY(hipMemcpy(dtv, tv.data(), tv.size(), hipMemcpyHostToDevice));
            P.bm_th = dth; P.bm_tv = dtv;
        } else P.bm_cols[e->nlevels] = 0;
    }
    if ((rc = dev_alloc(e, &P.cell_count, B * cells))) return rc;
    if ((rc = dev_alloc(e, &P.cell_list, B * P.cell_list_frame_stride))) return rc;
    if ((rc = dev_alloc(e, &P.keys, B * keys))) return rc;
    if ((rc = dev_alloc(e, &P.node_of, B * keys))) return rc;
    if ((rc = dev_alloc(e, &P.lvl_kp, B * kps))) return rc;
    if ((rc = dev_alloc(e, &P.lvl_perm, B * kps))) return rc;
    if ((rc = dev_alloc(e, &P.lvl_angle, B * kps))) return rc;
    if ((rc = dev_alloc(e, &P.lvl_desc, B * kps * 32))) return rc;
    if ((rc = dev_alloc(e, &P.lvl_count, B * e->nlevels))) return rc;
    if ((rc = dev_alloc(e, &P.lvl_ncand, B * e->nlevels))) return rc;
    if ((rc = dev_alloc(e, &P.status, 1))) return rc;
    {
        auto up = [](size_t v) { return (v + 255) & ~(size_t)255; };
        e->ob_kp = up(8 * B); e->ob_desc = e->ob_kp + up(sizeof(orbhip_keypoint) * B * P.max_kp);
        e->outblob_bytes = e->ob_desc + up((size_t)32 * B * P.max_kp);
        if ((rc = dev_alloc(e, &e->d_outblob, e->outblob_bytes))) return rc;
        P.out_count = reinterpret_cast<int32_t *>(e->d_outblob); P.out_mono = P.out_count + B;
        P.out_kp = reinterpret_cast<orbhip_keypoint *>(e->d_outblob + e->ob_kp); P.out_desc = e->d_outblob + e->ob_desc;
    }
    HIP_TRY(hipMemset(P.status, 0, sizeof(int32_t)));
    P.oct_nc = orb_octree_nc(P);
    if (orb_octree_lds_bytes(P.oct_nc) > 150 * 1024) { g_last_error = "per-level quota (or nIni) too large for the LDS-resident octree"; return ORBHIP_E_BADARG; }
    if ((rc = orb_lds_optin(orb_octree_func(), e->ctx->device, orb_octree_lds_bytes(P.oct_nc)))) return rc;
    if ((rc = orb_lds_optin(orb_fast_cells_func(e->F.small_cells), e->ctx->device, sizeof(uint32_t) * (size_t)e->F.wave_dw))) return rc;
    if (e->F.use_runs && (rc = orb_lds_optin(orb_fast_runs_func((e->F.run_rows - 7) * 5 <= 256 ? 4 : 6), e->ctx->device, sizeof(uint32_t) * (size_t)e->F.run_dw))) return rc;
    e->width = width; e->height = height; e->max_batch = max_batch;
    return ORBHIP_OK;
}

extern "C" int orbhip_compute_stereo_matches_device(orbhip_extractor *left, orbhip_extractor *right, float mb, float mbf,
                                                    float *d_u_right, float *d_depth, int32_t *d_n_matches)
{
    if (!left || !right || !d_u_right || !d_depth || !(mb > 0) || !(mbf > 0)) return ORBHIP_E_BADARG;
    if (!left->max_batch || !right->max_batch || left->last_batch <= 0 || left->last_batch != right->last_batch ||
        left->width != right->width || left->height != right->height || left->nlevels != right->nlevels ||
        left->scale_factor != right->scale_factor || left->P.max_kp != right->P.max_kp || left->P.max_kp > 65535) {
        g_last_error = "stereo: extractors must share geometry, feature budget and batch, and have extracted";
        return ORBHIP_E_BADARG;
    }
    HIP_TRY(hipSetDevice(left->ctx->device));
    if (!left->d_stereo_sad) {
        int rc = dev_alloc(left, &left->d_stereo_sad, (size_t)left->max_batch * left->P.max_kp);
        if (rc) return rc;
    }
    if (right->ctx->stream != left->ctx->stream) {
        hipEvent_t ev;
        HIP_TRY(hipEventCreateWithFlags(&ev, hipEventDisableTiming));
        HIP_TRY(hipEventRecord(ev, right->ctx->stream));
        HIP_TRY(hipStreamWaitEvent(left->ctx->stream, ev, 0));
        HIP_TRY(hipEventDestroy(ev));
    }
    StereoArgs A;
    memset(&A, 0, sizeof(A));
    for (int l = 0; l < left->nlevels; l++) {
        const OrbLevel &a = left->P.lv[l], &b = right->P.lv[l];
        A.lv[l].imgL = a.img; A.lv[l].imgR = b.img; A.lv[l].fsL = a.img_frame_stride; A.lv[l].fsR = b.img_frame_stride;
        A.lv[l].pitchL = a.img_pitch; A.lv[l].pitchR = b.img_pitch; A.lv[l].wR = b.w;
        A.lv[l].scale = left->scale[l]; A.lv[l].inv_scale = left->inv_scale[l];
    }
    A.nlevels = left->nlevels; A.batch = left->last_batch; A.max_kp = left->P.max_kp; A.rows0 = left->height;
    A.kpL = left->P.out_kp; A.kpR = right->P.out_kp; A.descL = left->P.out_desc; A.descR = right->P.out_desc;
    A.nL = left->P.out_count; A.nR = right->P.out_count;
    A.mb = mb; A.mbf = mbf; A.u_right = d_u_right; A.depth = d_depth; A.sad = left->d_stereo_sad; A.n_kept = d_n_matches;
    orb_launch_stereo(A, left->ctx->stream);
    HIP_TRY(hipGetLastError());
    if (right->ctx->stream != left->ctx->stream) {
        hipEvent_t ev;
        HIP_TRY(hipEventCreateWithFlags(&ev, hipEventDisableTiming));
        HIP_TRY(hipEventRecord(ev, left->ctx->stream));
        HIP_TRY(hipStreamWaitEvent(right->ctx->stream, ev, 0));
        HIP_TRY(hipEventDestroy(ev));
    }
    return ORBHIP_OK;
}

extern "C" int orbhip_compute_stereo_matches_host(orbhip_extractor *left, orbhip_extractor *right, float mb, float mbf,
                                                  float *u_right_out, float *depth_out, int n, int32_t *n_matches_out)
{
    if (!left || !right || n < 0 || (n && (!u_right_out || !depth_out))) return ORBHIP_E_BADARG;
    if (n_matches_out) *n_matches_out = 0;
    for (int i = 0; i < n; i++) { u_right_out[i] = -1.0f; depth_out[i] = -1.0f; }
    if (n == 0) return ORBHIP_OK;
    if (left->last_batch <= 0 || n > left->P.max_kp) { g_last_error = "stereo: the left extractor holds no extraction of that many keypoints"; return ORBHIP_E_BADARG; }
    const size_t slots = (size_t)left->max_batch * left->P.max_kp;
    uint8_t *w = (uint8_t *)orbhip_ctx_work_internal(left->ctx, 8 * slots + 4 * (size_t)left->max_batch + 256);
    if (!w) return ORBHIP_E_HIP;
    float *d_ur = (float *)w, *d_dp = d_ur + slots;
    int32_t *d_nk = (int32_t *)(d_dp + slots);
    const int rc = orbhip_compute_stereo_matches_device(left, right, mb, mbf, d_ur, d_dp, d_nk);
    if (rc) return rc;
    uint8_t *h = (uint8_t *)orbhip_ctx_pinned_internal(left->ctx, 8 * (size_t)n + 16);
    if (!h) return ORBHIP_E_HIP;
    hipStream_t st = left->ctx->stream;
    HIP_TRY(hipMemcpyAsync(h, d_ur, 4 * (size_t)n, hipMemcpyDeviceToHost, st));
    HIP_TRY(hipMemcpyAsync(h + 4 * (size_t)n, d_dp, 4 * (size_t)n, hipMemcpyDeviceToHost, st));
    HIP_TRY(hipMemcpyAsync(h + 8 * (size_t)n, d_nk, 4, hipMemcpyDeviceToHost, st));
    HIP_TRY(hipStreamSynchronize(st));
    memcpy(u_right_out, h, 4 * (size_t)n); memcpy(depth_out, h + 4 * (size_t)n, 4 * (size_t)n);
    if (n_matches_out) memcpy(n_matches_out, h + 8 * (size_t)n, 4);
    return ORBHIP_OK;
}

extern "C" int orbhip_compute_stereo_fisheye_matches_host(orbhip_extractor *left, orbhip_extractor *right, int cam1_type, const float *cam1,
        int cam2_type, const float *cam2, const float *Rlr, const float *tlr, const float *level_sigma2, int nlevels,
        int32_t *l2r_out, float *depth_out, float *x3d_out, int n_left, int32_t *r2l_out, int n_right, int32_t *n_matches_out)
{
    if (!left || !right || n_left < 0 || n_right < 0 || (n_left && (!l2r_out || !depth_out || !x3d_out)) || (n_right && !r2l_out)) return ORBHIP_E_BADARG;
    if (n_matches_out) *n_matches_out = 0;
    for (int i = 0; i < n_left; i++) { l2r_out[i] = -1; depth_out[i] = -1.0f; x3d_out[3 * i] = x3d_out[3 * i + 1] = x3d_out[3 * i + 2] = 0.0f; }
    for (int i = 0; i < n_right; i++) r2l_out[i] = -1;
    if (n_left == 0) return ORBHIP_OK;
    const orbhip_keypoint *dk, *hk; const uint8_t *dd, *hd; int32_t cl = -1, cr = -1;
    if (orbhip_extractor_last_frame(left, 0, &dk, &dd, &hk, &hd, &cl, nullptr) != ORBHIP_OK || cl != n_left ||
        orbhip_extractor_last_frame(right, 0, &dk, &dd, &hk, &hd, &cr, nullptr) != ORBHIP_OK || cr != n_right) {
        g_last_error = "stereo fisheye: n_left / n_right are not the counts of the extractors' latest host extractions";
        return ORBHIP_E_BADARG;
    }
    if (left->ctx->device != right->ctx->device) { g_last_error = "stereo fisheye: extractors on two devices"; return ORBHIP_E_BADARG; }
    HIP_TRY(hipSetDevice(left->ctx->device));
    const int max_n = std::max(n_left, n_right);
    const size_t words = 6 * (size_t)max_n + 1;
    int32_t *w = (int32_t *)orbhip_ctx_work_internal(left->ctx, 4 * words + 256);
    if (!w) return ORBHIP_E_HIP;
    int32_t *d_l2r = w, *d_r2l = w + max_n, *d_nm = w + 6 * (size_t)max_n;
    float *d_dp = (float *)(w + 2 * (size_t)max_n), *d_x = (float *)(w + 3 * (size_t)max_n);
    hipStream_t st = left->ctx->stream;
    if (right->ctx->stream != st) {
        hipEvent_t ev;
        HIP_TRY(hipEventCreateWithFlags(&ev, hipEventDisableTiming));
        HIP_TRY(hipEventRecord(ev, right->ctx->stream));
        HIP_TRY(hipStreamWaitEvent(st, ev, 0));
        HIP_TRY(hipEventDestroy(ev));
    }
    const int rc = orbhip_compute_stereo_fisheye_matches_device(left->ctx, left->P.out_kp, left->P.out_desc, left->P.out_count, left->P.out_mono,
                                                                 left->P.max_kp, right->P.out_kp, right->P.out_desc, right->P.out_count,
                                                                 right->P.out_mono, right->P.max_kp, 1, max_n, cam1_type, cam1, cam2_type, cam2, Rlr,
                                                                 tlr, level_sigma2, nlevels, d_l2r, d_r2l, d_dp, d_x, d_nm);
    if (rc) return rc;
    if (right->ctx->stream != st) {
        hipEvent_t ev;
        HIP_TRY(hipEventCreateWithFlags(&ev, hipEventDisableTiming));
        HIP_TRY(hipEventRecord(ev, st));
        HIP_TRY(hipStreamWaitEvent(right->ctx->stream, ev, 0));
        HIP_TRY(hipEventDestroy(ev));
    }
    int32_t *h = (int32_t *)orbhip_ctx_pinned_internal(left->ctx, 4 * words + 16);
    if (!h) return ORBHIP_E_HIP;
    HIP_TRY(hipMemcpyAsync(h, w, 4 * words, hipMemcpyDeviceToHost, st));
    HIP_TRY(hipStreamSynchronize(st));
    memcpy(l2r_out, h, 4 * (size_t)n_left);
    if (n_right) memcpy(r2l_out, h + max_n, 4 * (size_t)n_right);
    memcpy(depth_out, h + 2 * (size_t)max_n, 4 * (size_t)n_left);
    memcpy(x3d_out, h + 3 * (size_t)max_n, 12 * (size_t)n_left);
    if (n_matches_out) *n_matches_out = h[6 * (size_t)max_n];
    return ORBHIP_OK;
}

extern "C" int orbhip_extractor_blur_kernel(const orbhip_extractor *e, int batch)
{
    if (!e || !e->max_batch) return -1;
    const OrbParams &P = e->P;
    if (P.bm_cols[e->nlevels] > 0 && batch >= P.bm_min_batch) return 2;
    if (P.br_blocks[e->nlevels] > 0 && batch >= P.rows_min_batch) return 1;
    return 0;
}

extern "C" int orbhip_extractor_resize_band_rows(const orbhip_extractor *e, int level)
{
    if (!e || !e->max_batch || level < 1 || level >= e->nlevels) return -1;
    return e->P.lv[level].xchunk ? e->P.lv[level].rs_rows : 0;
}

extern "C" int orbhip_extractor_set_profiling(orbhip_extractor *e, int enable)
{
    if (!e) return ORBHIP_E_BADARG;
    if (enable && !e->ev_created) {
        for (auto &slot : e->ev) for (auto &ev : slot) HIP_TRY(hipEventCreate(&ev));
        e->ev_created = true;
    }
    e->profiling = enable != 0;
    e->ev_calls = 0;
    return ORBHIP_OK;
}

extern "C" int orbhip_extractor_stage_ms(orbhip_extractor *e, float *ms_out)
{
    if (!e || !ms_out || !e->ev_created || e->ev_calls <= 0) return ORBHIP_E_BADARG;
    const int n = std::min(e->ev_calls, ORBHIP_PROF_SLOTS);
    for (int i = 0; i < ORBHIP_STAGE_COUNT; i++) ms_out[i] = 0.f;
    for (int c = 0; c < n; c++) {
        const int slot = (e->ev_calls - 1 - c) % ORBHIP_PROF_SLOTS;
        HIP_TRY(hipEventSynchronize(e->ev[slot][ORBHIP_STAGE_COUNT]));
        for (int i = 0; i < ORBHIP_STAGE_COUNT; i++) {
            float ms = 0.f;
            HIP_TRY(hipEventElapsedTime(&ms, e->ev[slot][i], e->ev[slot][i + 1]));
            ms_out[i] += ms / n;
        }
    }
    e->ev_calls = 0;
    return ORBHIP_OK;
}

static int tune_int(const char *name, int dflt) { const char *v = getenv(name); return v ? atoi(v) : dflt; }

static int run_pipeline(orbhip_extractor *e, int batch, int lap0, int lap1)
{
    OrbParams &P = e->P;
    P.batch = batch; P.lap0 = lap0; P.lap1 = lap1; P.n_cus = e->ctx->n_cus;
    hipStream_t s = e->ctx->stream;
    const bool prof = e->profiling;
    const int slot = e->ev_calls % ORBHIP_PROF_SLOTS;
#define STAGE_MARK(i) do { if (prof) HIP_TRY(hipEventRecord(e->ev[slot][i], s)); } while (0)
    const bool fork = e->overlap && !prof && batch >= ORB_OVERLAP_MIN_BATCH;
    if (fork && !e->aux_ok) {
        HIP_TRY(hipStreamCreateWithFlags(&e->aux, hipStreamNonBlocking));
        HIP_TRY(hipEventCreateWithFlags(&e->ev_fork, hipEventDisableTiming));
        HIP_TRY(hipEventCreateWithFlags(&e->ev_join, hipEventDisableTiming));
        HIP_TRY(hipEventCreateWithFlags(&e->ev_pyr, hipEventDisableTiming));
        e->aux_ok = true;
    }
    FastParams &F = e->F;
    for (int l = 0; l < e->nlevels; l++) { F.lv[l].img = P.lv[l].img; F.lv[l].frame_stride = P.lv[l].img_frame_stride; F.lv[l].img_pitch = P.lv[l].img_pitch; }
    F.batch = batch; F.n_cus = e->ctx->n_cus; F.cell_count = P.cell_count; F.cell_list = P.cell_list; F.cell_list_frame_stride = P.cell_list_frame_stride; F.status = P.status;
    const bool rows = P.br_blocks[e->nlevels] > 0 && batch >= P.rows_min_batch;
    const int fast_waves = fork ? tune_int("ORBHIP_TUNE_FAST_WAVES", rows ? 18 : 10) : 0;
    STAGE_MARK(ORBHIP_STAGE_PYRAMID);
    if (fork && e->nlevels > 1 && rows && tune_int("ORBHIP_TUNE_L0_EARLY", 0)) {
        HIP_TRY(hipEventRecord(e->ev_fork, s));
        HIP_TRY(hipStreamWaitEvent(e->aux, e->ev_fork, 0));
        orb_launch_fast_cells(F, s, fast_waves, 0, 1);
        for (int l = 1; l < e->nlevels; l++) orb_launch_resize(P, l, e->aux);
        HIP_TRY(hipEventRecord(e->ev_pyr, e->aux));
        HIP_TRY(hipStreamWaitEvent(s, e->ev_pyr, 0));
        orb_launch_fast_cells(F, s, fast_waves, 1, e->nlevels);
        orb_launch_blur(P, e->aux, 5);
        HIP_TRY(hipEventRecord(e->ev_join, e->aux));
    } else {
        for (int l = 1; l < e->nlevels; l++) orb_launch_resize(P, l, s);
        STAGE_MARK(ORBHIP_STAGE_FAST_CELLS);
        if (fork) {
            HIP_TRY(hipEventRecord(e->ev_fork, s));
            HIP_TRY(hipStreamWaitEvent(e->aux, e->ev_fork, 0));
        }
        orb_launch_fast_cells(F, s, fast_waves);
        if (fork) {
            if (!tune_int("ORBHIP_TUNE_SKIP_BLUR", 0))
                orb_launch_blur(P, e->aux, tune_int("ORBHIP_TUNE_BLUR_WGS", 5));
            HIP_TRY(hipEventRecord(e->ev_join, e->aux));
        }
    }
    STAGE_MARK(ORBHIP_STAGE_BLUR);
    if (!fork) orb_launch_blur(P, s, 8);
    STAGE_MARK(ORBHIP_STAGE_OCTREE);
    orb_launch_octree(P, s);
    STAGE_MARK(ORBHIP_STAGE_DESC);
    if (fork) HIP_TRY(hipStreamWaitEvent(s, e->ev_join, 0));
    orb_launch_orient_desc(P, s);
    STAGE_MARK(ORBHIP_STAGE_ASSEMBLE);
    orb_launch_assemble(P, s);
    STAGE_MARK(ORBHIP_STAGE_COUNT);
#undef STAGE_MARK
    if (prof) e->ev_calls++;
    HIP_TRY(hipGetLastError());
    e->last_batch = batch;
    e->generation++;
    return ORBHIP_OK;
}

static int run_pipeline_graph(orbhip_extractor *e, int width, int height, int batch, int lap0, int lap1)
{
    if (!(e->graph_valid && e->g_w == width && e->g_h == height && e->g_batch == batch && e->g_lap0 == lap0 && e->g_lap1 == lap1)) {
        if (e->graph_valid) { (void)hipGraphExecDestroy(e->graph_exec); e->graph_valid = false; }
        hipGraph_t graph = nullptr;
        HIP_TRY(hipStreamBeginCapture(e->ctx->stream, hipStreamCaptureModeThreadLocal));
        const int rc = run_pipeline(e, batch, lap0, lap1);
        hipError_t ce = hipStreamEndCapture(e->ctx->stream, &graph);
        if (rc) { if (graph) (void)hipGraphDestroy(graph); return rc; }
        if (ce != hipSuccess) { g_last_error = std::string("hipStreamEndCapture: ") + hipGetErrorString(ce); return ORBHIP_E_HIP; }
        hipError_t ie = hipGraphInstantiate(&e->graph_exec, graph, nullptr, nullptr, 0);
        (void)hipGraphDestroy(graph);
        if (ie != hipSuccess) { g_last_error = std::string("hipGraphInstantiate: ") + hipGetErrorString(ie); return ORBHIP_E_HIP; }
        e->graph_valid = true; e->g_w = width; e->g_h = height; e->g_batch = batch; e->g_lap0 = lap0; e->g_lap1 = lap1;
    }
    HIP_TRY(hipGraphLaunch(e->graph_exec, e->ctx->stream));
    e->last_batch = batch;
    e->generation++;
    return ORBHIP_OK;
}

extern "C" int orbhip_extract_batch_device(orbhip_extractor *e, const uint8_t *d_images, int width, int height,
                                           size_t row_stride, size_t frame_stride, int batch, int lap0, int lap1)
{
    if (!e || batch <= 0 || row_stride < (size_t)width) return ORBHIP_E_BADARG;
    if (!d_images || width <= 0 || height <= 0) return ORBHIP_E_EMPTY;
    HIP_TRY(hipSetDevice(e->ctx->device));
    int rc = orbhip_extractor_reserve(e, width, height, batch);
    if (rc) return rc;
    OrbLevel &L0 = e->P.lv[0];
    const bool aligned = ((uintptr_t)d_images % 4 == 0) && (row_stride % 4 == 0) && (frame_stride % 4 == 0);
    const bool use_graph = e->graph_mode && !e->profiling;
    if (aligned && !use_graph) {
        L0.img = const_cast<uint8_t *>(d_images);
        L0.img_pitch = (int)row_stride;
        L0.img_frame_stride = frame_stride;
    } else {
        L0.img = e->d_level0; L0.img_pitch = e->level0_pitch; L0.img_frame_stride = e->level0_frame_stride;
        for (int f = 0; f < batch; f++)
            HIP_TRY(hipMemcpy2DAsync(L0.img + (size_t)f * L0.img_frame_stride, L0.img_pitch, d_images + (size_t)f * frame_stride,
                                     row_stride, width, height, hipMemcpyDeviceToDevice, e->ctx->stream));
    }
    return use_graph ? run_pipeline_graph(e, width, height, batch, lap0, lap1) : run_pipeline(e, batch, lap0, lap1);
}

extern "C" int orbhip_extractor_set_graph_mode(orbhip_extractor *e, int enable)
{
    if (!e) return ORBHIP_E_BADARG;
    e->graph_mode = enable != 0;
    if (!e->graph_mode && e->graph_valid) { (void)hipGraphExecDestroy(e->graph_exec); e->graph_valid = false; }
    return ORBHIP_OK;
}

extern "C" int orbhip_extractor_results(orbhip_extractor *e, orbhip_keypoint **d_kp, uint8_t **d_desc,
                                        int32_t **d_count, int32_t **d_mono)
{
    if (!e || !e->max_batch) return ORBHIP_E_BADARG;
    if (d_kp) *d_kp = e->P.out_kp;
    if (d_desc) *d_desc = e->P.out_desc;
    if (d_count) *d_count = e->P.out_count;
    if (d_mono) *d_mono = e->P.out_mono;
    return ORBHIP_OK;
}

static int extract_host_core(orbhip_extractor *e, const uint8_t *h_images, int width, int height, size_t row_stride, size_t frame_stride,
                             int batch, int lap0, int lap1)
{
    if (!e || batch <= 0) return ORBHIP_E_BADARG;
    if (!h_images || width <= 0 || height <= 0) return ORBHIP_E_EMPTY;
    if (row_stride < (size_t)width) return ORBHIP_E_BADARG;
    HIP_TRY(hipSetDevice(e->ctx->device));
    int rc = orbhip_extractor_reserve(e, width, height, batch);
    if (rc) return rc;
    hipStream_t s = e->ctx->stream;
    OrbLevel &L0 = e->P.lv[0];
    L0.img = e->d_level0; L0.img_pitch = e->level0_pitch; L0.img_frame_stride = e->level0_frame_stride;
    const size_t in_bytes = (size_t)batch * L0.img_frame_stride;
    if (e->h_in_bytes < in_bytes) {
        if (e->h_in) (void)hipHostFree(e->h_in);
        e->h_in = nullptr; e->h_in_bytes = 0;
        HIP_TRY(hipHostMalloc((void **)&e->h_in, (size_t)e->max_batch * L0.img_frame_stride, hipHostMallocDefault));
        e->h_in_bytes = (size_t)e->max_batch * L0.img_frame_stride;
    }
    if (!e->h_out) HIP_TRY(hipHostMalloc((void **)&e->h_out, e->outblob_bytes, hipHostMallocDefault));
    if (!e->h_status) HIP_TRY(hipHostMalloc((void **)&e->h_status, 256, hipHostMallocDefault));
    for (int f = 0; f < batch; f++) {
        const uint8_t *src = h_images + (size_t)f * frame_stride;
        uint8_t *dst = e->h_in + (size_t)f * L0.img_frame_stride;
        if (row_stride == (size_t)L0.img_pitch) memcpy(dst, src, (size_t)L0.img_pitch * (height - 1) + width);
        else for (int y = 0; y < height; y++) memcpy(dst + (size_t)y * L0.img_pitch, src + (size_t)y * row_stride, width);
    }
    HIP_TRY(hipMemcpyAsync(L0.img, e->h_in, in_bytes, hipMemcpyHostToDevice, s));
    e->view_generation = ~0ull;
    rc = (e->graph_mode && !e->profiling) ? run_pipeline_graph(e, width, height, batch, lap0, lap1) : run_pipeline(e, batch, lap0, lap1);
    if (rc) return rc;
    const size_t B = (size_t)e->max_batch, mk = (size_t)e->P.max_kp;
    if ((size_t)batch == B) HIP_TRY(hipMemcpyAsync(e->h_out, e->d_outblob, e->outblob_bytes, hipMemcpyDeviceToHost, s));
    else {
        HIP_TRY(hipMemcpyAsync(e->h_out, e->d_outblob, 8 * B, hipMemcpyDeviceToHost, s));
        HIP_TRY(hipMemcpyAsync(e->h_out + e->ob_kp, e->d_outblob + e->ob_kp, sizeof(orbhip_keypoint) * mk * batch, hipMemcpyDeviceToHost, s));
        HIP_TRY(hipMemcpyAsync(e->h_out + e->ob_desc, e->d_outblob + e->ob_desc, 32 * mk * batch, hipMemcpyDeviceToHost, s));
    }
    HIP_TRY(hipMemcpyAsync(e->h_status, e->P.status, sizeof(int32_t), hipMemcpyDeviceToHost, s));
    HIP_TRY(hipStreamSynchronize(s));
    if (*e->h_status) {
        g_last_error = "device-side list capacity exceeded";
        (void)hipMemsetAsync(e->P.status, 0, sizeof(int32_t), s);
        return *e->h_status;
    }
    e->view_generation = e->generation;
    return ORBHIP_OK;
}

extern "C" int orbhip_extract_batch_host(orbhip_extractor *e, const uint8_t *h_images, int width, int height,
                                         size_t row_stride, size_t frame_stride, int batch, int lap0, int lap1,
                                         orbhip_keypoint *kp_out, uint8_t *desc_out, int cap,
                                         int32_t *count_out, int32_t *mono_out)
{
    if (e && batch > 0 && h_images && width > 0 && height > 0 && (!kp_out || !desc_out || !count_out || !mono_out)) return ORBHIP_E_BADARG;
    const int rc = extract_host_core(e, h_images, width, height, row_stride, frame_stride, batch, lap0, lap1);
    if (rc) return rc;
    const int32_t *cnt = reinterpret_cast<const int32_t *>(e->h_out), *mono = cnt + e->max_batch;
    const size_t mk = (size_t)e->P.max_kp;
    for (int f = 0; f < batch; f++) {
        count_out[f] = cnt[f]; mono_out[f] = mono[f];
        if (cnt[f] > cap) return ORBHIP_E_CAPACITY;
        if (cnt[f] == 0) continue;
        memcpy(kp_out + (size_t)f * cap, e->h_out + e->ob_kp + sizeof(orbhip_keypoint) * mk * f, sizeof(orbhip_keypoint) * cnt[f]);
        memcpy(desc_out + (size_t)f * cap * 32, e->h_out + e->ob_desc + 32 * mk * f, (size_t)32 * cnt[f]);
    }
    return ORBHIP_OK;
}

extern "C" int orbhip_extract_batch_host_view(orbhip_extractor *e, const uint8_t *h_images, int width, int height, size_t row_stride,
                                              size_t frame_stride, int batch, int lap0, int lap1, const orbhip_keypoint **kp_view,
                                              const uint8_t **desc_view, int *row_capacity, const int32_t **count_view, const int32_t **mono_view)
{
    if (e && batch > 0 && h_images && width > 0 && height > 0 && (!kp_view || !desc_view || !row_capacity || !count_view || !mono_view)) return ORBHIP_E_BADARG;
    const int rc = extract_host_core(e, h_images, width, height, row_stride, frame_stride, batch, lap0, lap1);
// ... 161 lines not shown
```

orb-slam3-mac_amd/python/orbhip.py:

```python
import ctypes as C
import os
import numpy as np

try:
    import torch
except Exception:
    torch = None

_HERE = os.path.dirname(os.path.abspath(__file__))
LIB_DIR = os.path.join(os.path.dirname(_HERE), "lib")
LIB_PATH = os.path.join(LIB_DIR, "liborbhip.so")
SYNTH_PATH = os.path.join(LIB_DIR, "libsynth.so")

if not os.path.exists(LIB_PATH):
    raise ImportError(
        "liborbhip.so not built: run `python -c 'import __graft_entry__ as g; g.build()'` "
        "(there is no CPU fallback for the HIP path)")

lib = C.CDLL(LIB_PATH)

OK, E_BADARG, E_NODEVICE, E_HIP, E_CAPACITY, E_ABORTED, E_NOTSPD, E_EMPTY = 0, -1, -2, -3, -4, -5, -6, -7
STAGES = ["pyramid", "fast_cells", "blur", "octree", "desc", "assemble"]

KP_DTYPE = np.dtype([("x", "<f4"), ("y", "<f4"), ("size", "<f4"), ("angle", "<f4"),
                     ("response", "<f4"), ("octave", "<i4"), ("class_id", "<i4")])
assert KP_DTYPE.itemsize == 28

vp, ci, cf, cd, sz = C.c_void_p, C.c_int, C.c_float, C.c_double, C.c_size_t
lib.orbhip_version.restype = C.c_char_p
lib.orbhip_last_error.restype = C.c_char_p
lib.orbhip_ctx_create.argtypes = [ci, vp, C.POINTER(vp)]
lib.orbhip_ctx_destroy.argtypes = [vp]
lib.orbhip_ctx_synchronize.argtypes = [vp]
lib.orbhip_ctx_stream.argtypes = [vp]
lib.orbhip_ctx_stream.restype = vp
lib.orbhip_extractor_create.argtypes = [vp, ci, cf, ci, ci, ci, C.POINTER(vp)]
lib.orbhip_extractor_destroy.argtypes = [vp]
lib.orbhip_extractor_levels.argtypes = [vp]
lib.orbhip_extractor_table.argtypes = [vp, ci, vp]
lib.orbhip_extractor_features_per_level.argtypes = [vp, vp]
lib.orbhip_extractor_umax.argtypes = [vp, vp]
lib.orbhip_extractor_reserve.argtypes = [vp, ci, ci, ci]
lib.orbhip_extractor_max_keypoints.argtypes = [vp]
lib.orbhip_extract_batch_device.argtypes = [vp, vp, ci, ci, sz, sz, ci, ci, ci]
lib.orbhip_extractor_results.argtypes = [vp, C.POINTER(vp), C.POINTER(vp), C.POINTER(vp), C.POINTER(vp)]
lib.orbhip_extract_batch_host.argtypes = [vp, vp, ci, ci, sz, sz, ci, ci, ci, vp, vp, ci, vp, vp]
lib.orbhip_extractor_level_dims.argtypes = [vp, ci, C.POINTER(ci), C.POINTER(ci)]
lib.orbhip_extractor_get_pyramid_level.argtypes = [vp, ci, ci, ci, vp, sz]
lib.orbhip_extractor_get_blurred_level.argtypes = [vp, ci, ci, vp, sz]
lib.orbhip_extractor_get_pyramid_padded.argtypes = [vp, ci, vp, vp]
lib.orbhip_extractor_get_fast_candidates.argtypes = [vp, ci, ci, vp, vp, vp, ci, C.POINTER(C.c_int32)]
lib.orbhip_extractor_get_level_keypoints.argtypes = [vp, ci, ci, vp, ci, C.POINTER(C.c_int32)]
lib.orbhip_extractor_set_profiling.argtypes = [vp, ci]
lib.orbhip_extractor_set_graph_mode.argtypes = [vp, ci]
lib.orbhip_extractor_stage_ms.argtypes = [vp, vp]
lib.orbhip_descriptor_distance.argtypes = [vp, vp]
lib.orbhip_match_bf2nn_device.argtypes = [vp, vp, vp, sz, vp, vp, sz, ci, ci, cd, vp, vp, vp]
lib.orbhip_search_for_initialization_device.argtypes = [vp, vp, vp, vp, vp, vp, vp, ci, ci, sz, cf, cf, cf, cf, ci, cf, ci,
                                                        vp, vp, vp]
lib.orbhip_ctx_check_status.argtypes = [vp]
lib.orbhip_ctx_wait_for.argtypes = [vp, vp]
lib.orbhip_extractor_blur_kernel.argtypes = [vp, ci]
lib.orbhip_extractor_blur_kernel.restype = ci
lib.orbhip_extractor_resize_band_rows.argtypes = [vp, ci]
lib.orbhip_extractor_resize_band_rows.restype = ci
lib.orbhip_prev_matched_init_device.argtypes = [vp, vp, sz, ci, ci, vp]
lib.orbhip_search_by_projection_device.argtypes = [vp, vp, vp, vp, ci, vp, vp, vp, vp, ci, sz, ci, cf, cf, cf, cf, ci, ci, vp, vp]
lib.orbhip_search_local_map_device.argtypes = [vp, vp, vp, vp, ci, vp, vp, vp, vp, ci, sz, ci, cf, cf, cf, cf, ci, cf, vp, vp]


class OrbHipError(RuntimeError):
    def __init__(self, code, where):
        self.code = code
        super().__init__("%s failed: %d (%s)" % (where, code, lib.orbhip_last_error().decode()))


def _chk(rc, where):
    if rc != OK:
        raise OrbHipError(rc, where)


class Context:
    def __init__(self, device=0, stream=None):
        h = vp()
        _chk(lib.orbhip_ctx_create(device, stream, C.byref(h)), "orbhip_ctx_create")
        self.h = h

    def synchronize(self):
        _chk(lib.orbhip_ctx_synchronize(self.h), "orbhip_ctx_synchronize")

    def check_status(self):
        _chk(lib.orbhip_ctx_check_status(self.h), "orbhip_ctx_check_status")

    def wait_for(self, other):
        _chk(lib.orbhip_ctx_wait_for(self.h, other.h), "orbhip_ctx_wait_for")

    @property
    def stream(self):
        return lib.orbhip_ctx_stream(self.h)

    def close(self):
        if self.h:
            lib.orbhip_ctx_destroy(self.h)
            self.h = None


class Extractor:

    def __init__(self, ctx, nfeatures=1000, scale_factor=1.2, nlevels=8, ini_th=20, min_th=7):
        h = vp()
        _chk(lib.orbhip_extractor_create(ctx.h, nfeatures, scale_factor, nlevels, ini_th, min_th, C.byref(h)),
             "orbhip_extractor_create")
        self.h, self.ctx, self.nlevels = h, ctx, nlevels

    def close(self):
        if self.h:
            lib.orbhip_extractor_destroy(self.h)
            self.h = None

    def table(self, which):
        out = np.zeros(self.nlevels, np.float32)
        _chk(lib.orbhip_extractor_table(self.h, which, out.ctypes.data), "orbhip_extractor_table")
        return out

    def features_per_level(self):
        out = np.zeros(self.nlevels, np.int32)
        _chk(lib.orbhip_extractor_features_per_level(self.h, out.ctypes.data), "features_per_level")
        return out

    def umax(self):
        out = np.zeros(16, np.int32)
        _chk(lib.orbhip_extractor_umax(self.h, out.ctypes.data), "umax")
        return out

    def reserve(self, w, h, batch):
        _chk(lib.orbhip_extractor_reserve(self.h, w, h, batch), "orbhip_extractor_reserve")

    @property
    def max_keypoints(self):
        return lib.orbhip_extractor_max_keypoints(self.h)

    def blur_kernel(self, batch):
        return ("k_blur", "k_blur_rows", "k_blur_mfma")[lib.orbhip_extractor_blur_kernel(self.h, int(batch))]

    def resize_band_rows(self, level):
        return lib.orbhip_extractor_resize_band_rows(self.h, int(level))

    def set_graph_mode(self, on):
        _chk(lib.orbhip_extractor_set_graph_mode(self.h, 1 if on else 0), "orbhip_extractor_set_graph_mode")

    def set_profiling(self, on):
        _chk(lib.orbhip_extractor_set_profiling(self.h, 1 if on else 0), "set_profiling")

    def stage_ms(self):
        out = np.zeros(len(STAGES), np.float32)
        _chk(lib.orbhip_extractor_stage_ms(self.h, out.ctypes.data), "stage_ms")
        return dict(zip(STAGES, out.tolist()))

    def extract_host(self, images, lap=(0, 1000)):
        img = np.ascontiguousarray(images, np.uint8)
        if img.ndim == 2:
            img = img[None]
        B, H, W = img.shape
        self.reserve(W, H, B)
        cap = self.max_keypoints
        kp = np.zeros((B, cap), KP_DTYPE)
        desc = np.zeros((B, cap, 32), np.uint8)
        cnt = np.zeros(B, np.int32)
        mono = np.zeros(B, np.int32)
        _chk(lib.orbhip_extract_batch_host(self.h, img.ctypes.data, W, H, W, W * H, B, lap[0], lap[1],
                                           kp.ctypes.data, desc.ctypes.data, cap, cnt.ctypes.data, mono.ctypes.data),
             "orbhip_extract_batch_host")
        return [(kp[f, :cnt[f]].copy(), desc[f, :cnt[f]].copy(), int(mono[f])) for f in range(B)]

    def extract_device(self, d_ptr, w, h, row_stride, frame_stride, batch, lap=(0, 1000)):
        _chk(lib.orbhip_extract_batch_device(self.h, d_ptr, w, h, row_stride, frame_stride, batch, lap[0], lap[1]),
             "orbhip_extract_batch_device")

    def results_device(self):
        a, b, c, d = vp(), vp(), vp(), vp()
        _chk(lib.orbhip_extractor_results(self.h, C.byref(a), C.byref(b), C.byref(c), C.byref(d)), "results")
        return a.value, b.value, c.value, d.value

    def level_dims(self, level):
        w, h = ci(), ci()
        _chk(lib.orbhip_extractor_level_dims(self.h, level, C.byref(w), C.byref(h)), "level_dims")
        return w.value, h.value

    def pyramid_level(self, frame, level, padded=False):
        w, h = self.level_dims(level)
        if padded:
            w, h = w + 38, h + 38
        out = np.zeros((h, w), np.uint8)
        _chk(lib.orbhip_extractor_get_pyramid_level(self.h, frame, level, 1 if padded else 0, out.ctypes.data, w),
             "get_pyramid_level")
        return out

    def pyramid_padded(self, frame):
        outs = [np.zeros((h + 38, w + 38), np.uint8) for w, h in (self.level_dims(l) for l in range(self.nlevels))]
        ptrs = (vp * self.nlevels)(*[o.ctypes.data for o in outs])
        strides = (C.c_size_t * self.nlevels)(*[o.shape[1] for o in outs])
        _chk(lib.orbhip_extractor_get_pyramid_padded(self.h, frame, ptrs, strides), "get_pyramid_padded")
        return outs

    def blurred_level(self, frame, level):
        w, h = self.level_dims(level)
        out = np.zeros((h, w), np.uint8)
        _chk(lib.orbhip_extractor_get_blurred_level(self.h, frame, level, out.ctypes.data, w), "get_blurred_level")
        return out

    def fast_candidates(self, frame, level, cap=1 << 17):
        xs, ys, ss = (np.zeros(cap, np.int32) for _ in range(3))
        n = C.c_int32()
        _chk(lib.orbhip_extractor_get_fast_candidates(self.h, frame, level, xs.ctypes.data, ys.ctypes.data,
                                                      ss.ctypes.data, cap, C.byref(n)), "get_fast_candidates")
        return xs[:n.value].copy(), ys[:n.value].copy(), ss[:n.value].copy()

    def level_keypoints(self, frame, level, cap=8192):
        out = np.zeros(cap, KP_DTYPE)
        n = C.c_int32()
        _chk(lib.orbhip_extractor_get_level_keypoints(self.h, frame, level, out.ctypes.data, cap, C.byref(n)),
             "get_level_keypoints")
        return out[:n.value].copy()


def match_bf2nn_device(ctx, d_descA, d_nA, strideA, d_descB, d_nB, strideB, pairs, max_n, ratio, d_idx2, d_dist2,
                       d_accept):
    _chk(lib.orbhip_match_bf2nn_device(ctx.h, d_descA, d_nA, strideA, d_descB, d_nB, strideB, pairs, max_n, ratio,
                                       d_idx2, d_dist2, d_accept), "orbhip_match_bf2nn_device")


def search_for_initialization_device(ctx, d_kpA, d_descA, d_nA, d_kpB, d_descB, d_nB, pairs, max_n, kp_stride, bounds,
                                     window, nn_ratio, check_ori, d_prev, d_m12, d_nmatches):
    _chk(lib.orbhip_search_for_initialization_device(ctx.h, d_kpA, d_descA, d_nA, d_kpB, d_descB, d_nB, pairs, max_n,
                                                     kp_stride, bounds[0], bounds[1], bounds[2], bounds[3], window,
                                                     nn_ratio, 1 if check_ori else 0, d_prev, d_m12, d_nmatches),
         "orbhip_search_for_initialization_device")


PROJ_QUERY_DTYPE = np.dtype([("u", np.float32), ("v", np.float32), ("radius", np.float32), ("ur", np.float32),
                             ("angle", np.float32), ("min_level", np.int32), ("max_level", np.int32), ("has_obs", np.int32)])


def search_by_projection_device(ctx, d_q, d_desc_q, d_nq, max_q, d_kp, d_desc, d_u_right, d_n, max_n, kp_stride, pairs,
                                bounds, th_high, check_ori, d_train_match, d_nmatches):
    _chk(lib.orbhip_search_by_projection_device(ctx.h, d_q, d_desc_q, d_nq, max_q, d_kp, d_desc, d_u_right, d_n, max_n,
                                                kp_stride, pairs, bounds[0], bounds[1], bounds[2], bounds[3], th_high,
                                                1 if check_ori else 0, d_train_match, d_nmatches),
         "orbhip_search_by_projection_device")


def search_local_map_device(ctx, d_q, d_desc_q, d_nq, max_q, d_kp, d_desc, d_u_right, d_n, max_n, kp_stride, pairs,
                            bounds, th_high, nn_ratio, d_train_match, d_nmatches):
    _chk(lib.orbhip_search_local_map_device(ctx.h, d_q, d_desc_q, d_nq, max_q, d_kp, d_desc, d_u_right, d_n, max_n,
                                            kp_stride, pairs, bounds[0], bounds[1], bounds[2], bounds[3], th_high,
                                            nn_ratio, d_train_match, d_nmatches), "orbhip_search_local_map_device")


def prev_matched_init_device(ctx, d_kp, kp_stride, frames, max_n, d_prev):
    _chk(lib.orbhip_prev_matched_init_device(ctx.h, d_kp, kp_stride, frames, max_n, d_prev), "orbhip_prev_matched_init_device")


def descriptor_distance(a, b):
    a = np.ascontiguousarray(a, np.uint8)
    b = np.ascontiguousarray(b, np.uint8)
    return lib.orbhip_descriptor_distance(a.ctypes.data, b.ctypes.data)


_synth = None


def synth_lib():
    global _synth
    if _synth is None:
        _synth = C.CDLL(SYNTH_PATH)
        _synth.synth_frame.argtypes = [vp, ci, ci, ci, C.c_uint64, ci]
        _synth.synth_batch.argtypes = [vp, ci, ci, ci, C.c_uint64, ci]
        _synth.synth_frame_transform.argtypes = [C.c_uint64, ci, C.POINTER(cf), C.POINTER(cf), C.POINTER(cf)]
    return _synth


def synth_frames(w, h, n, seed=20241004, first=0):
    out = np.zeros((n, h, w), np.uint8)
    synth_lib().synth_batch(out.ctypes.data, w, h, n, seed, first)
    return out


def rig2_fields(g):
    r = g.get("rig2")
    if r is None:
        return ((cd * 7)(0, 0, 0, 0, 0, 0, 0), 0.0, 0.0, 0.0, 0.0, 0, (cd * 4)(0, 0, 0, 0))
    kb2 = r.get("kb")
    return ((cd * 7)(*r["Trl"]), *[float(c) for c in r["cam"]], 1 if kb2 is not None else 0, (cd * 4)(*(kb2 if kb2 is not None else (0, 0, 0, 0))))


class BaCamera(C.Structure):
    _fields_ = [("fx", cd), ("fy", cd), ("cx", cd), ("cy", cd), ("bf", cd), ("camera_model", C.c_int32), ("kb", cd * 4),
                ("Trl", cd * 7), ("fx2", cd), ("fy2", cd), ("cx2", cd), ("cy2", cd), ("camera2_model", C.c_int32), ("kb2", cd * 4)]


class BaGraph(C.Structure):
    _fields_ = [("n_poses", C.c_int32), ("n_points", C.c_int32), ("n_edges", C.c_int32),
                ("pose_fixed", vp), ("edge_pose", vp), ("edge_point", vp), ("edge_obs", vp),
                ("edge_inv_sigma2", vp), ("edge_stereo", vp),
                ("fx", cd), ("fy", cd), ("cx", cd), ("cy", cd), ("bf", cd),
                ("camera_model", C.c_int32), ("kb", cd * 4),
                ("Trl", cd * 7), ("fx2", cd), ("fy2", cd), ("cx2", cd), ("cy2", cd), ("camera2_model", C.c_int32), ("kb2", cd * 4),
                ("n_cameras", C.c_int32), ("cameras", vp), ("pose_camera", vp)]


def camera_table(g, cls=None):
    cls = cls or BaCamera
    cams = g.get("cameras")
    if not cams:
        return 0, None, None
    arr = (cls * len(cams))()
    for i, c in enumerate(cams):
        kb = c.get("kb")
        arr[i] = cls(c["fx"], c["fy"], c["cx"], c["cy"], c["bf"], 1 if kb is not None else 0, (cd * 4)(*(kb if kb is not None else (0, 0, 0, 0))),
                     *rig2_fields(dict(rig2=c.get("rig2"))))
    return len(cams), arr, np.ascontiguousarray(g["pose_camera"], np.int32)


class BaParams(C.Structure):
    _fields_ = [("iters1", C.c_int32), ("iters2", C.c_int32), ("huber_mono2", cd), ("huber_stereo2", cd),
                ("user_lambda_init", cd), ("tau", cd), ("max_trials", C.c_int32),
                ("stage2_exclude_outliers", C.c_int32), ("stage2_drop_robust", C.c_int32), ("no_discard", C.c_int32),
                ("gate_mono2", cd), ("gate_stereo2", cd)]


class BaStats(C.Structure):
    _fields_ = [("iterations_run", C.c_int32 * 2), ("lm_trials", C.c_int32), ("n_outliers", C.c_int32),
                ("discarded", C.c_int32), ("chi2_initial", cd), ("chi2_final", cd)]

    def as_dict(self):
        return dict(iterations_run=list(self.iterations_run), lm_trials=self.lm_trials, n_outliers=self.n_outliers,
                    discarded=self.discarded, chi2_initial=self.chi2_initial, chi2_final=self.chi2_final)


lib.orbhip_ba_default_params.argtypes = [C.POINTER(BaParams)]
lib.orbhip_ba_merge_params.argtypes = [C.POINTER(BaParams)]
lib.orbhip_ba_batch_create.argtypes = [vp, vp, ci, vp, vp, C.POINTER(vp)]
lib.orbhip_ba_batch_solve.argtypes = [vp, C.POINTER(BaParams), vp]
lib.orbhip_ba_batch_download.argtypes = [vp, vp, vp, vp, vp]
lib.orbhip_ba_batch_ticks.argtypes = [vp]
lib.orbhip_ba_batch_destroy.argtypes = [vp]
lib.orbhip_ba_solve_batch.argtypes = [vp, vp, ci, C.POINTER(BaParams), vp, vp, vp, vp, vp]
lib.orbhip_ba_batch_set_profiling.argtypes = [vp, ci]
lib.orbhip_ba_batch_gemm_profile.argtypes = [vp, C.POINTER(cf), C.POINTER(ci), C.POINTER(cd)]
lib.orbhip_mfma_f64_peak_tflops.argtypes = [vp, C.POINTER(cd)]
lib.orbhip_ba_batch_gemm_dense_flops.argtypes = [vp]
lib.orbhip_ba_batch_gemm_issued_flops.argtypes = [vp]
lib.orbhip_ba_batch_gemm_issued_flops.restype = cd
lib.orbhip_ba_batch_gemm_dense_flops.restype = cd


def mfma_f64_peak_tflops(ctx):
    v = cd()
    _chk(lib.orbhip_mfma_f64_peak_tflops(ctx.h, C.byref(v)), "orbhip_mfma_f64_peak_tflops")
    return v.value


lib.orbhip_ctx_set_ba_schur_mode.argtypes = [vp, ci]


def ba_set_schur_mode(ctx, mode):
    _chk(lib.orbhip_ctx_set_ba_schur_mode(ctx.h, mode), "orbhip_ctx_set_ba_schur_mode")


def ba_merge_params():
    p = BaParams()
    lib.orbhip_ba_merge_params(C.byref(p))
    return p


def ba_global_params(iterations, robust=True):
# ... 529 lines not shown
```

Baseline: 315,300 frames/s.

## Template octree kernel on team size and split levels into per-team groups

```diff
diff --git a/include/orbhip.h b/include/orbhip.h
--- a/include/orbhip.h
+++ b/include/orbhip.h
@@ -60,6 +60,12 @@
 int orbhip_extractor_blur_kernel(const orbhip_extractor *ext, int batch);
 
 int orbhip_extractor_resize_band_rows(const orbhip_extractor *ext, int level);
+
+int orbhip_extractor_octree_team(const orbhip_extractor *ext, int level, int batch);
+int orbhip_extractor_octree_caps(const orbhip_extractor *ext, int level, int *node_cap, int *key_cap);
+int orbhip_octree_team_slots(int team);
+int orbhip_octree_plan_query(int nlevels, const int *node_cap, const int *key_cap, int batch, int force_team,
+                             int *team_of_level, long long *groups);
 
 int orbhip_extractor_last_frame(orbhip_extractor *ext, int frame, const orbhip_keypoint **d_kp, const uint8_t **d_desc,
                                 const orbhip_keypoint **h_kp_view, const uint8_t **h_desc_view, int32_t *count, unsigned long long *generation);
diff --git a/orb-slam3-mac_amd/csrc/orb_internal.h b/orb-slam3-mac_amd/csrc/orb_internal.h
--- a/orb-slam3-mac_amd/csrc/orb_internal.h
+++ b/orb-slam3-mac_amd/csrc/orb_internal.h
@@ -41,6 +41,9 @@
     int kps_per_frame;
     int max_kp;
     int oct_nc;
+    int oct_team_force;
+    int oct_nc64, oct_kc64;
+    int oct_nc128, oct_kc128;
     int rows_min_batch;
     int bm_min_batch;
     int br_blocks[ORB_MAX_LEVELS + 1];
@@ -124,9 +127,20 @@
 #endif
 void orb_launch_blur(const OrbParams &P, hipStream_t s, int wgs_per_cu, int frame0 = 0, int nframes = -1);
 const void *orb_fast_cells_func(int small);
-void orb_launch_octree(const OrbParams &P, hipStream_t s);
+#define ORB_OCT_MAX_GROUPS 3
+struct OctGroup { int team, nlv, nc; unsigned long long lvls; };
+int orb_octree_plan(const OrbParams &P, int batch, OctGroup *g);
+int orb_octree_team(const OrbParams &P, int level, int batch);
+int orb_octree_level_nc(const OrbParams &P, int level);
+int orb_octree_rule_from_env(OrbParams &P);
+#define ORB_OCT_NC64 0
+#define ORB_OCT_KC64 0
+#define ORB_OCT_NC128 0
+#define ORB_OCT_KC128 0
+int orb_octree_slots(int team);
+void orb_launch_octree(const OrbParams &P, const OctGroup &g, hipStream_t s);
 void orb_launch_orient_desc(const OrbParams &P, hipStream_t s);
 void orb_launch_assemble(const OrbParams &P, hipStream_t s);
 size_t orb_octree_lds_bytes(int nc);
 int orb_octree_nc(const OrbParams &P);
-const void *orb_octree_func();
+const void *orb_octree_func(int team);
diff --git a/orb-slam3-mac_amd/csrc/orb_kernels.hip b/orb-slam3-mac_amd/csrc/orb_kernels.hip
--- a/orb-slam3-mac_amd/csrc/orb_kernels.hip
+++ b/orb-slam3-mac_amd/csrc/orb_kernels.hip
@@ -797,10 +797,16 @@
     uint32_t *best;
 };
 
+int orb_octree_level_nc(const OrbParams &P, int l)
+{
+    const int a = P.lv[l].quota + 16, b = 4 * P.lv[l].n_ini + 4;
+    return a > b ? a : b;
+}
+
 int orb_octree_nc(const OrbParams &P)
 {
     int nc = 0;
-    for (int l = 0; l < P.nlevels; l++) { const int a = P.lv[l].quota + 16, b = 4 * P.lv[l].n_ini + 4; nc = a > nc ? a : nc; nc = b > nc ? b : nc; }
+    for (int l = 0; l < P.nlevels; l++) { const int a = orb_octree_level_nc(P, l); nc = a > nc ? a : nc; }
     return nc;
 }
 
@@ -817,10 +823,36 @@
     return (kx < mx ? 0 : 1) + (ky < my ? 0 : 2);
 }
 
-#define OCT_KR 8
+template <int T> __device__ __forceinline__ void team_sync()
+{
+    if constexpr (T == WAVE) {
+        __builtin_amdgcn_fence(__ATOMIC_RELEASE, "workgroup"); __builtin_amdgcn_wave_barrier(); __builtin_amdgcn_fence(__ATOMIC_ACQUIRE, "workgroup");
+    } else __syncthreads();
+}
+template <int T> __device__ __forceinline__ int team_excl_scan(int v, int *wsum, int *total)
+{
+    const int inc = wave_incl_scan(v);
+    if constexpr (T == WAVE) {
+        *total = __builtin_amdgcn_readlane(inc, WAVE - 1);
+        return inc - v;
+    } else {
+        const int lane = threadIdx.x & (WAVE - 1), wid = threadIdx.x >> 6;
+        if (lane == WAVE - 1) wsum[wid] = inc;
+        __syncthreads();
+        int base = 0, tot = 0;
+#pragma unroll
+        for (int w = 0; w < T / WAVE; w++) { const int s = wsum[w]; if (w < wid) base += s; tot += s; }
+        *total = tot;
+        __syncthreads();
+        return base + inc - v;
+    }
+}
+
 #ifdef OCT_PROF
 __device__ long long g_oct_prof[8];
 #define OCT_T(i) do { if (blockIdx.x == 0 && threadIdx.x == 0) { const long long t_ = clock64(); g_oct_prof[i] += t_ - t_prev; t_prev = t_; } } while (0)
+#define OCT_R0() const long long r0_ = clock64()
+#define OCT_R(i) do { if (blockIdx.x == 0 && threadIdx.x == 0) g_oct_prof[i] += clock64() - r0_; } while (0)
 extern "C" int orbhip_debug_oct_prof(long long *out8, int reset)
 {
     if (out8 && hipMemcpyFromSymbol(out8, HIP_SYMBOL(g_oct_prof), 64) != hipSuccess) return -1;
@@ -829,21 +861,33 @@
 }
 #else
 #define OCT_T(i) do { } while (0)
+#define OCT_R0() do { } while (0)
+#define OCT_R(i) do { } while (0)
 #endif
-__global__ __launch_bounds__(256) void k_octree(OrbParams P)
-{
-    extern __shared__ uint32_t smem[];
-    __shared__ int wsum[8];
-    __shared__ int s_size, s_front, s_nexpand, s_rstar, s_T, s_nproc;
+#ifndef OCT_PACKED_RANKS
+#define OCT_PACKED_RANKS 0
+#endif
+#ifndef OCT_EARLY_EXIT_256
+#define OCT_EARLY_EXIT_256 0
+#endif
+#define OCT_EARLY_EXIT(T) ((T) < 256 || OCT_EARLY_EXIT_256)
+static_assert(ORB_MAX_LEVELS <= 16, "k_octree's level list holds 16 levels of 4 bits");
+template <int T, int KR>
+__global__ __launch_bounds__(T) void k_octree(OrbParams P, int NC, unsigned long long lvls)
+{
+    extern __shared__ __align__(16) uint32_t oct_smem[];
+    uint32_t *smem = oct_smem;
+    __shared__ int wsum[4];
+    __shared__ int s_size, s_front, s_nexpand, s_rstar;
     const int tid = threadIdx.x;
 #ifdef OCT_PROF
     long long t_prev = clock64();
 #endif
-    const int lvl = blockIdx.x / P.batch;
-    const int frame = blockIdx.x - lvl * P.batch;
+    const int gi = blockIdx.x / P.batch;
+    const int frame = blockIdx.x - gi * P.batch;
+    const int lvl = (int)((lvls >> (4 * gi)) & 15);
     const OrbLevel &L = P.lv[lvl];
     const int N = L.quota;
-    const int NC = P.oct_nc;
     uint32_t *box0 = smem, *box1 = smem + NC, *cnt = smem + 2 * NC;
     uint32_t *nbox0 = smem + 3 * NC, *nbox1 = smem + 4 * NC, *ncnt = smem + 5 * NC;
     OctLds S;
@@ -858,21 +902,21 @@
     uint32_t *keys = P.keys + (size_t)frame * P.keys_per_frame + L.key_base;
     uint16_t *node_of = P.node_of + (size_t)frame * P.keys_per_frame + L.key_base;
     const int ncells = L.ncols * L.nrows;
-    uint32_t rk[OCT_KR]; int rn[OCT_KR];
+    uint32_t rk[KR]; int rn[KR];
     int running = 0;
     int32_t *count_out = P.lvl_count + frame * P.nlevels + lvl;
     if (ncells + 1 <= 16 * NC) {
         int *coff = reinterpret_cast<int *>(smem);
-        for (int c0 = 0; c0 < ncells; c0 += 256) {
+        for (int c0 = 0; c0 < ncells; c0 += T) {
             const int c = c0 + tid;
             const int n = c < ncells ? min((int)ccount[c], L.cell_cap) : 0;
             int total;
-            const int off = running + block_excl_scan256(n, wsum, &total);
+            const int off = running + team_excl_scan<T>(n, wsum, &total);
             if (c < ncells) coff[c] = off;
             running += total;
         }
         if (tid == 0) coff[ncells] = running;
-        __syncthreads();
+        team_sync<T>();
         if (running > L.key_cap) { if (tid == 0) atomicExch(P.status, ORBHIP_E_CAPACITY); running = L.key_cap; }
         const int K0 = running;
         auto fetch = [&](int k) {
@@ -881,50 +925,54 @@
             return clist[(size_t)lo * L.cell_cap + (k - coff[lo])];
         };
 #pragma unroll
-        for (int i = 0; i < OCT_KR; i++) { const int k = tid + 256 * i; rk[i] = k < K0 ? fetch(k) : 0u; rn[i] = 0; }
-#pragma unroll
-        for (int i = 0; i < OCT_KR; i++) { const int k = tid + 256 * i; if (k < K0) keys[k] = rk[i]; }
-        for (int k = tid + 256 * OCT_KR; k < K0; k += 256) keys[k] = fetch(k);
-        __syncthreads();
+        for (int i = 0; i < KR; i++) { rk[i] = 0u; rn[i] = 0; }
+#pragma unroll
+        for (int i = 0; i < KR; i++) { const int k = tid + T * i; if (OCT_EARLY_EXIT(T) && T * i >= K0) break; if (k < K0) rk[i] = fetch(k); }
+#pragma unroll
+        for (int i = 0; i < KR; i++) { const int k = tid + T * i; if (OCT_EARLY_EXIT(T) && T * i >= K0) break; if (k < K0) keys[k] = rk[i]; }
+        for (int k = tid + T * KR; k < K0; k += T) keys[k] = fetch(k);
+        team_sync<T>();
     } else {
-        for (int c0 = 0; c0 < ncells; c0 += 256) {
+        for (int c0 = 0; c0 < ncells; c0 += T) {
             const int c = c0 + tid;
             const int n = c < ncells ? (int)ccount[c] : 0;
             int total;
-            const int off = running + block_excl_scan256(n, wsum, &total);
+            const int off = running + team_excl_scan<T>(n, wsum, &total);
             for (int i = 0; i < n; i++)
                 if (off + i < L.key_cap) keys[off + i] = clist[(size_t)c * L.cell_cap + i];
             running += total;
         }
         if (running > L.key_cap) { if (tid == 0) atomicExch(P.status, ORBHIP_E_CAPACITY); running = L.key_cap; }
-        __syncthreads();
+        team_sync<T>();
         __threadfence_block();
 #pragma unroll
-        for (int i = 0; i < OCT_KR; i++) { const int k = tid + 256 * i; rk[i] = k < running ? keys[k] : 0u; rn[i] = 0; }
+        for (int i = 0; i < KR; i++) { const int k = tid + T * i; rk[i] = k < running ? keys[k] : 0u; rn[i] = 0; }
     }
     const int K = running;
     if (tid == 0) P.lvl_ncand[frame * P.nlevels + lvl] = K;
     if (K == 0) { if (tid == 0) *count_out = 0; return; }
-    __syncthreads();
+    team_sync<T>();
     __threadfence_block();
     OCT_T(0);
     const int n_ini = L.n_ini;
     const int H = (L.h - ORB_MINB) - ORB_MINB;
-    for (int i = tid; i < NC; i += 256) { cnt[i] = 0; ncnt[i] = 0; }
-    __syncthreads();
-#pragma unroll
-    for (int i = 0; i < OCT_KR; i++)
-        if (tid + 256 * i < K) {
+    for (int i = tid; i < NC; i += T) { cnt[i] = 0; ncnt[i] = 0; }
+    team_sync<T>();
+#pragma unroll
+    for (int i = 0; i < KR; i++) {
+        if (OCT_EARLY_EXIT(T) && T * i >= K) break;
+        if (tid + T * i < K) {
             const int r = (int)__fdiv_rn((float)ORB_KEY_X(rk[i]), L.hx);
             rn[i] = r;
             atomicAdd(&ncnt[r], 1u);
         }
-    for (int k = tid + 256 * OCT_KR; k < K; k += 256) {
+    }
+    for (int k = tid + T * KR; k < K; k += T) {
         const int r = (int)__fdiv_rn((float)ORB_KEY_X(keys[k]), L.hx);
         node_of[k] = (uint16_t)r;
         atomicAdd(&ncnt[r], 1u);
     }
-    __syncthreads();
+    team_sync<T>();
     if (tid == 0) {
         int m = 0;
         for (int i = 0; i < n_ini; i++) {
@@ -939,42 +987,62 @@
         }
         s_size = m; s_front = m;
     }
-    __syncthreads();
-#pragma unroll
-    for (int i = 0; i < OCT_KR; i++) if (tid + 256 * i < K) rn[i] = S.newpos[rn[i]];
-    for (int k = tid + 256 * OCT_KR; k < K; k += 256) node_of[k] = (uint16_t)S.newpos[node_of[k]];
-    __syncthreads();
+    team_sync<T>();
+#pragma unroll
+    for (int i = 0; i < KR; i++) { if (OCT_EARLY_EXIT(T) && T * i >= K) break; if (tid + T * i < K) rn[i] = S.newpos[rn[i]]; }
+    for (int k = tid + T * KR; k < K; k += T) node_of[k] = (uint16_t)S.newpos[node_of[k]];
+    team_sync<T>();
 
     OCT_T(1);
     bool final_phase = false;
     int size = s_size, front = s_front;
+    const bool packed = OCT_PACKED_RANKS && NC <= 2048;
+    uint32_t *const fk = smem + ((6 * NC + 3) & ~3);
     for (int guard = 0; guard < 64; guard++) {
         int C;
         if (!final_phase) {
             int run = 0;
-            for (int p0 = 0; p0 < size; p0 += 256) {
+            for (int p0 = 0; p0 < size; p0 += T) {
                 const int p = p0 + tid;
                 const int f = (p < size && cnt[p] > 1) ? 1 : 0;
                 int tot;
-                const int o = run + block_excl_scan256(f, wsum, &tot);
+                const int o = run + team_excl_scan<T>(f, wsum, &tot);
                 if (p < size) { S.ord[p] = f ? o : -1; if (f) S.by_ord[o] = p; }
                 run += tot;
             }
             C = run;
         } else {
             int run = 0;
-            for (int p0 = 0; p0 < size; p0 += 256) {
+            for (int p0 = 0; p0 < size; p0 += T) {
                 const int p = p0 + tid;
                 const int f = (p < front && cnt[p] > 1) ? 1 : 0;
                 int tot;
-                const int o = run + block_excl_scan256(f, wsum, &tot);
+                const int o = run + team_excl_scan<T>(f, wsum, &tot);
                 if (p < size) S.ord[p] = -1;
-                if (f) S.excl[o] = p;
+                if (f) {
+                    S.excl[o] = p;
+                    if (packed) fk[o] = ((0xFFFFFu - cnt[p]) << 11) | (uint32_t)o;
+                }
                 run += tot;
             }
             C = run;
-            __syncthreads();
-            for (int i = tid; i < C; i += 256) {
+            if (packed && tid < 4 && C + tid < ((C + 3) & ~3)) fk[C + tid] = 0xFFFFFFFFu;
+            team_sync<T>();
+            OCT_R0();
+            if (packed) {
+                for (int i = tid; i < C; i += T) {
+                    const uint32_t ki = fk[i];
+                    int r = 0;
+                    for (int j = 0; j < C; j += 4) {
+                        const uint4 q = *reinterpret_cast<const uint4 *>(&fk[j]);
+                        r += (q.x < ki) + (q.y < ki) + (q.z < ki) + (q.w < ki);
+                    }
+                    const int p = S.excl[i];
+                    S.ord[p] = r;
+                    S.by_ord[r] = p;
+                }
+            } else
+            for (int i = tid; i < C; i += T) {
                 const int p = S.excl[i];
                 const uint32_t ci = cnt[p];
                 int r = 0;
@@ -985,31 +1053,34 @@
                 S.ord[p] = r;
                 S.by_ord[r] = p;
             }
-        }
-        __syncthreads();
+            OCT_R(6);
+        }
+        team_sync<T>();
         if (C == 0) break;
-        for (int i = tid; i < 4 * size; i += 256) S.cc[i] = 0;
+        for (int i = tid; i < 4 * size; i += T) S.cc[i] = 0;
         if (tid == 0) { s_nexpand = 0; s_rstar = C - 1; }
-        __syncthreads();
-#pragma unroll
-        for (int i = 0; i < OCT_KR; i++)
-            if (tid + 256 * i < K) {
+        team_sync<T>();
+#pragma unroll
+        for (int i = 0; i < KR; i++) {
+            if (OCT_EARLY_EXIT(T) && T * i >= K) break;
+            if (tid + T * i < K) {
                 const int p = rn[i];
                 if (S.ord[p] >= 0) atomicAdd(&S.cc[4 * p + oct_quadrant(rk[i], box0[p], box1[p])], 1u);
             }
-        for (int k = tid + 256 * OCT_KR; k < K; k += 256) {
+        }
+        for (int k = tid + T * KR; k < K; k += T) {
             const int p = node_of[k];
             if (S.ord[p] >= 0) atomicAdd(&S.cc[4 * p + oct_quadrant(keys[k], box0[p], box1[p])], 1u);
         }
-        __syncthreads();
+        team_sync<T>();
         {
             int run = 0;
-            for (int o0 = 0; o0 < C; o0 += 256) {
+            for (int o0 = 0; o0 < C; o0 += T) {
                 const int o = o0 + tid;
                 int nch = 0;
                 if (o < C) { const uint32_t *q = &S.cc[4 * S.by_ord[o]]; nch = (q[0] > 0) + (q[1] > 0) + (q[2] > 0) + (q[3] > 0); }
                 int tot;
-                const int e = run + block_excl_scan256(nch, wsum, &tot);
+                const int e = run + team_excl_scan<T>(nch, wsum, &tot);
                 if (o < C) {
                     S.excl[o] = e;
                     if (final_phase && size + e + nch - (o + 1) >= N) atomicMin(&s_rstar, o);
@@ -1017,31 +1088,31 @@
                 run += tot;
             }
         }
-        __syncthreads();
+        team_sync<T>();
         const int rstar = s_rstar;
-        int T, nproc;
+        int Tn, nproc;
         {
             const uint32_t *q = &S.cc[4 * S.by_ord[rstar]];
-            T = S.excl[rstar] + (q[0] > 0) + (q[1] > 0) + (q[2] > 0) + (q[3] > 0);
+            Tn = S.excl[rstar] + (q[0] > 0) + (q[1] > 0) + (q[2] > 0) + (q[3] > 0);
             nproc = rstar + 1;
         }
         {
             int run = 0;
-            for (int p0 = 0; p0 < size; p0 += 256) {
+            for (int p0 = 0; p0 < size; p0 += T) {
                 const int p = p0 + tid;
                 const int surv = (p < size && !(S.ord[p] >= 0 && S.ord[p] <= rstar)) ? 1 : 0;
                 int tot;
-                const int e = run + block_excl_scan256(surv, wsum, &tot);
-                if (p < size && surv) S.newpos[p] = T + e;
+                const int e = run + team_excl_scan<T>(surv, wsum, &tot);
+                if (p < size && surv) S.newpos[p] = Tn + e;
                 run += tot;
             }
         }
-        for (int p = tid; p < size; p += 256) {
+        for (int p = tid; p < size; p += T) {
             const int o = S.ord[p];
             if (o >= 0 && o <= rstar) {
                 const uint32_t *q = &S.cc[4 * p];
                 const int nch = (q[0] > 0) + (q[1] > 0) + (q[2] > 0) + (q[3] > 0);
-                const int base = T - (S.excl[o] + nch);
+                const int base = Tn - (S.excl[o] + nch);
                 S.posbase[p] = base;
                 const uint32_t b0 = box0[p], b1 = box1[p];
                 const int x0 = b0 & 0xFFFF, y0 = b0 >> 16, x1 = b1 & 0xFFFF, y1 = b1 >> 16;
@@ -1064,7 +1135,7 @@
                 nbox0[np] = box0[p]; nbox1[np] = box1[p]; ncnt[np] = cnt[p];
             }
         }
-        __syncthreads();
+        team_sync<T>();
         auto relabel = [&](uint32_t key, int p) {
             const int o = S.ord[p];
             if (o >= 0 && o <= rstar) {
@@ -1077,56 +1148,127 @@
             return S.newpos[p];
         };
 #pragma unroll
-        for (int i = 0; i < OCT_KR; i++) if (tid + 256 * i < K) rn[i] = relabel(rk[i], rn[i]);
-        for (int k = tid + 256 * OCT_KR; k < K; k += 256) node_of[k] = (uint16_t)relabel(keys[k], node_of[k]);
-        __syncthreads();
-        const int new_size = T + (size - nproc);
+        for (int i = 0; i < KR; i++) { if (OCT_EARLY_EXIT(T) && T * i >= K) break; if (tid + T * i < K) rn[i] = relabel(rk[i], rn[i]); }
+        for (int k = tid + T * KR; k < K; k += T) node_of[k] = (uint16_t)relabel(keys[k], node_of[k]);
+        team_sync<T>();
+        const int new_size = Tn + (size - nproc);
         const int nexpand = s_nexpand;
         { uint32_t *t; t = box0; box0 = nbox0; nbox0 = t; t = box1; box1 = nbox1; nbox1 = t; t = cnt; cnt = ncnt; ncnt = t; }
         const int old_size = size;
-        size = new_size; front = T;
+        size = new_size; front = Tn;
 #ifdef OCT_PROF
         if (blockIdx.x == 0 && tid == 0) g_oct_prof[5] += 1;
 #endif
         if (new_size >= N || new_size == old_size) break;
         if (!final_phase && new_size + 3 * nexpand > N) final_phase = true;
     }
-    __syncthreads();
+    team_sync<T>();
     OCT_T(2);
-    for (int i = tid; i < size; i += 256) S.best[i] = 0;
-    __syncthreads();
-#pragma unroll
-    for (int i = 0; i < OCT_KR; i++)
-        if (tid + 256 * i < K) atomicMax(&S.best[rn[i]], ((uint32_t)ORB_KEY_S(rk[i]) << 20) | (uint32_t)(0xFFFFF - (tid + 256 * i)));
-    for (int k = tid + 256 * OCT_KR; k < K; k += 256)
+    for (int i = tid; i < size; i += T) S.best[i] = 0;
+    team_sync<T>();
+#pragma unroll
+    for (int i = 0; i < KR; i++) {
+        if (OCT_EARLY_EXIT(T) && T * i >= K) break;
+        if (tid + T * i < K) atomicMax(&S.best[rn[i]], ((uint32_t)ORB_KEY_S(rk[i]) << 20) | (uint32_t)(0xFFFFF - (tid + T * i)));
+    }
+    for (int k = tid + T * KR; k < K; k += T)
         atomicMax(&S.best[node_of[k]], ((uint32_t)ORB_KEY_S(keys[k]) << 20) | (uint32_t)(0xFFFFF - k));
-    __syncthreads();
+    team_sync<T>();
     OCT_T(3);
     uint32_t *out = P.lvl_kp + (size_t)frame * P.kps_per_frame + L.kp_base;
     int nout = size;
     if (nout > L.kp_cap) { if (tid == 0) atomicExch(P.status, ORBHIP_E_CAPACITY); nout = L.kp_cap; }
     uint16_t *perm = P.lvl_perm + (size_t)frame * P.kps_per_frame + L.kp_base;
-    for (int i = tid; i < nout; i += 256) out[i] = keys[0xFFFFF - (S.best[i] & 0xFFFFF)];
+    for (int i = tid; i < nout; i += T) out[i] = keys[0xFFFFF - (S.best[i] & 0xFFFFF)];
     if (P.batch < ORB_PERM_MIN_BATCH) { if (tid == 0) *count_out = nout; return; }
-    __syncthreads();
-    for (int i = tid; i < nout; i += 256) { const uint32_t ki = out[i]; S.best[i] = ((uint32_t)(ORB_KEY_Y(ki) >> 5) << 16) | (uint32_t)ORB_KEY_X(ki); }
-    __syncthreads();
-    for (int i = tid; i < nout; i += 256) {
+    if (packed) {
+        uint32_t *pk = smem;
+        for (int i = tid; i < ((nout + 3) & ~3); i += T) {
+            const uint32_t ki = i < nout ? out[i] : 0u;
+            pk[i] = i < nout ? ((uint32_t)(ORB_KEY_Y(ki) >> 5) << 23) | ((uint32_t)ORB_KEY_X(ki) << 11) | (uint32_t)i : 0xFFFFFFFFu;
+        }
+        team_sync<T>();
+        OCT_R0();
+        for (int i = tid; i < nout; i += T) {
+            const uint32_t si = pk[i];
+            int rank = 0;
+            for (int j = 0; j < nout; j += 4) {
+                const uint4 q = *reinterpret_cast<const uint4 *>(&pk[j]);
+                rank += (q.x < si) + (q.y < si) + (q.z < si) + (q.w < si);
+            }
+            perm[rank] = (uint16_t)i;
+        }
+        OCT_R(7);
+        if (tid == 0) *count_out = nout;
+        OCT_T(4);
+        return;
+    }
+    team_sync<T>();
+    for (int i = tid; i < nout; i += T) { const uint32_t ki = out[i]; S.best[i] = ((uint32_t)(ORB_KEY_Y(ki) >> 5) << 16) | (uint32_t)ORB_KEY_X(ki); }
+    team_sync<T>();
+    OCT_R0();
+    for (int i = tid; i < nout; i += T) {
         const uint32_t si = S.best[i];
         int rank = 0;
         for (int j = 0; j < nout; j++) { const uint32_t sj = S.best[j]; rank += (sj < si) || (sj == si && j < i); }
         perm[rank] = (uint16_t)i;
     }
+    OCT_R(7);
     if (tid == 0) *count_out = nout;
     OCT_T(4);
 }
 
-const void *orb_octree_func() { return reinterpret_cast<const void *>(k_octree); }
-
-void orb_launch_octree(const OrbParams &P, hipStream_t s)
-{
-    const size_t lds = orb_octree_lds_bytes(P.oct_nc);
-    hipLaunchKernelGGL(k_octree, dim3(P.nlevels * P.batch), dim3(256), lds, s, P);
+const void *orb_octree_func(int team)
+{
+    return team == 64 ? reinterpret_cast<const void *>(k_octree<64, 24>) : team == 128 ? reinterpret_cast<const void *>(k_octree<128, 12>)
+                                                                                     : reinterpret_cast<const void *>(k_octree<256, 8>);
+}
+
+int orb_octree_slots(int team) { return team == 256 ? 256 * 8 : 64 * 24; }
+
+int orb_octree_rule_from_env(OrbParams &P)
+{
+    auto env_int = [](const char *name, int dflt) { const char *v = getenv(name); return v && *v ? atoi(v) : dflt; };
+    P.oct_team_force = env_int("ORBHIP_OCTREE_TEAM", 0);
+    if (P.oct_team_force != 0 && P.oct_team_force != 64 && P.oct_team_force != 128 && P.oct_team_force != 256) return ORBHIP_E_BADARG;
+    P.oct_nc64 = env_int("ORBHIP_TUNE_OCT_NC64", ORB_OCT_NC64); P.oct_kc64 = env_int("ORBHIP_TUNE_OCT_KC64", ORB_OCT_KC64);
+    P.oct_nc128 = env_int("ORBHIP_TUNE_OCT_NC128", ORB_OCT_NC128); P.oct_kc128 = env_int("ORBHIP_TUNE_OCT_KC128", ORB_OCT_KC128);
+    return ORBHIP_OK;
+}
+
+int orb_octree_team(const OrbParams &P, int l, int batch)
+{
+    if (P.oct_team_force) return P.oct_team_force;
+    if (batch < ORB_OVERLAP_MIN_BATCH) return 256;
+    const int nc = orb_octree_level_nc(P, l), kc = P.lv[l].key_cap;
+    if (nc <= P.oct_nc64 && kc <= P.oct_kc64) return 64;
+    if (nc <= P.oct_nc128 && kc <= P.oct_kc128) return 128;
+    return 256;
+}
+
+int orb_octree_plan(const OrbParams &P, int batch, OctGroup *g)
+{
+    int n = 0;
+    for (int team = 256; team >= 64; team >>= 1) {
+        OctGroup G = {team, 0, 0, 0ull};
+        for (int l = 0; l < P.nlevels; l++)
+            if (orb_octree_team(P, l, batch) == team) {
+                G.lvls |= (unsigned long long)l << (4 * G.nlv++);
+                const int nc = orb_octree_level_nc(P, l);
+                G.nc = nc > G.nc ? nc : G.nc;
+            }
+        if (G.nlv) g[n++] = G;
+    }
+    return n;
+}
+
+void orb_launch_octree(const OrbParams &P, const OctGroup &G, hipStream_t s)
+{
+    const size_t lds = orb_octree_lds_bytes(G.nc);
+    const dim3 grid(G.nlv * P.batch);
+    if (G.team == 64) hipLaunchKernelGGL((k_octree<64, 24>), grid, dim3(64), lds, s, P, G.nc, G.lvls);
+    else if (G.team == 128) hipLaunchKernelGGL((k_octree<128, 12>), grid, dim3(128), lds, s, P, G.nc, G.lvls);
+    else hipLaunchKernelGGL((k_octree<256, 8>), grid, dim3(256), lds, s, P, G.nc, G.lvls);
 }
 
 #define BL_TW 64
diff --git a/orb-slam3-mac_amd/csrc/orbhip_api.hip b/orb-slam3-mac_amd/csrc/orbhip_api.hip
--- a/orb-slam3-mac_amd/csrc/orbhip_api.hip
+++ b/orb-slam3-mac_amd/csrc/orbhip_api.hip
@@ -224,6 +224,7 @@
     int32_t *d_stereo_sad;
     bool graph_mode, graph_valid;
     hipStream_t aux; hipEvent_t ev_fork, ev_join, ev_pyr; bool aux_ok; int overlap;
+    hipStream_t oct_aux[ORB_OCT_MAX_GROUPS - 1]; hipEvent_t ev_oct_fork, ev_oct_join[ORB_OCT_MAX_GROUPS - 1]; bool oct_aux_ok;
     hipGraphExec_t graph_exec;
     int g_w, g_h, g_batch, g_lap0, g_lap1;
     size_t level0_frame_stride; int level0_pitch;
@@ -246,6 +247,8 @@
     e->d_stereo_sad = nullptr;
     e->graph_mode = false; e->graph_valid = false; e->graph_exec = nullptr;
     e->aux = nullptr; e->ev_fork = e->ev_join = e->ev_pyr = nullptr; e->aux_ok = false; e->overlap = 1;
+    e->oct_aux_ok = false; e->ev_oct_fork = nullptr;
+    for (int i = 0; i < ORB_OCT_MAX_GROUPS - 1; i++) { e->oct_aux[i] = nullptr; e->ev_oct_join[i] = nullptr; }
     e->d_outblob = nullptr; e->outblob_bytes = e->ob_kp = e->ob_desc = 0; e->h_out = e->h_in = e->h_pyr = nullptr; e->h_in_bytes = e->h_pyr_bytes = 0; e->h_status = nullptr;
     e->generation = 0; e->view_generation = ~0ull;
     memset(&e->P, 0, sizeof(e->P));
@@ -286,6 +289,14 @@
 }
 static void ext_free_aux(orbhip_extractor *e)
 {
+    if (e->oct_aux_ok) {
+        for (int i = 0; i < ORB_OCT_MAX_GROUPS - 1; i++) {
+            if (e->oct_aux[i]) { (void)hipStreamSynchronize(e->oct_aux[i]); (void)hipStreamDestroy(e->oct_aux[i]); e->oct_aux[i] = nullptr; }
+            if (e->ev_oct_join[i]) { (void)hipEventDestroy(e->ev_oct_join[i]); e->ev_oct_join[i] = nullptr; }
+        }
+        if (e->ev_oct_fork) { (void)hipEventDestroy(e->ev_oct_fork); e->ev_oct_fork = nullptr; }
+        e->oct_aux_ok = false;
+    }
     if (!e->aux_ok) return;
     (void)hipStreamSynchronize(e->aux);
     (void)hipEventDestroy(e->ev_fork); (void)hipEventDestroy(e->ev_join); (void)hipEventDestroy(e->ev_pyr); (void)hipStreamDestroy(e->aux);
@@ -367,6 +378,7 @@
     OrbParams &P = e->P;
     memset(&P, 0, sizeof(P));
     P.nlevels = e->nlevels; P.ini_th = e->ini_th; P.min_th = e->min_th;
+    if (orb_octree_rule_from_env(P)) { g_last_error = "ORBHIP_OCTREE_TEAM must be 64, 128 or 256"; return ORBHIP_E_BADARG; }
     memcpy(P.umax, e->umax, sizeof(P.umax));
     memcpy(P.gauss_q8, e->gauss_q8, sizeof(P.gauss_q8));
     int cells = 0, keys = 0, kps = 0, max_cell_cap = 0;
@@ -615,7 +627,8 @@
     HIP_TRY(hipMemset(P.status, 0, sizeof(int32_t)));
     P.oct_nc = orb_octree_nc(P);
     if (orb_octree_lds_bytes(P.oct_nc) > 150 * 1024) { g_last_error = "per-level quota (or nIni) too large for the LDS-resident octree"; return ORBHIP_E_BADARG; }
-    if ((rc = orb_lds_optin(orb_octree_func(), e->ctx->device, orb_octree_lds_bytes(P.oct_nc)))) return rc;
+    for (int team = 64; team <= 256; team *= 2)
+        if ((rc = orb_lds_optin(orb_octree_func(team), e->ctx->device, orb_octree_lds_bytes(P.oct_nc)))) return rc;
     if ((rc = orb_lds_optin(orb_fast_cells_func(e->F.small_cells), e->ctx->device, sizeof(uint32_t) * (size_t)e->F.wave_dw))) return rc;
     if (e->F.use_runs && (rc = orb_lds_optin(orb_fast_runs_func((e->F.run_rows - 7) * 5 <= 256 ? 4 : 6), e->ctx->device, sizeof(uint32_t) * (size_t)e->F.run_dw))) return rc;
     e->width = width; e->height = height; e->max_batch = max_batch;
@@ -763,6 +776,44 @@
 {
     if (!e || !e->max_batch || level < 1 || level >= e->nlevels) return -1;
     return e->P.lv[level].xchunk ? e->P.lv[level].rs_rows : 0;
+}
+
+extern "C" int orbhip_extractor_octree_team(const orbhip_extractor *e, int level, int batch)
+{
+    if (!e || !e->max_batch || level < 0 || level >= e->nlevels || batch < 1) return -1;
+    return orb_octree_team(e->P, level, batch);
+}
+extern "C" int orbhip_extractor_octree_caps(const orbhip_extractor *e, int level, int *node_cap, int *key_cap)
+{
+    if (!e || !e->max_batch || level < 0 || level >= e->nlevels || !node_cap || !key_cap) return ORBHIP_E_BADARG;
+    *node_cap = orb_octree_level_nc(e->P, level); *key_cap = e->P.lv[level].key_cap;
+    return ORBHIP_OK;
+}
+extern "C" int orbhip_octree_team_slots(int team) { return team == 64 || team == 128 || team == 256 ? orb_octree_slots(team) : -1; }
+
+extern "C" int orbhip_octree_plan_query(int nlevels, const int *node_cap, const int *key_cap, int batch, int force_team,
+                                        int *team_of_level, long long *groups)
+{
+    if (nlevels < 1 || nlevels > ORB_MAX_LEVELS || !node_cap || !key_cap || batch < 1 || !team_of_level || !groups) return ORBHIP_E_BADARG;
+    if (force_team != 0 && force_team != 64 && force_team != 128 && force_team != 256) return ORBHIP_E_BADARG;
+    static OrbParams P;
+    static std::mutex mu;
+    std::lock_guard<std::mutex> lk(mu);
+    memset(&P, 0, sizeof(P));
+    P.nlevels = nlevels;
+    for (int l = 0; l < nlevels; l++) { P.lv[l].quota = node_cap[l] - 16; P.lv[l].n_ini = 1; P.lv[l].key_cap = key_cap[l]; }
+    P.oct_nc = orb_octree_nc(P);
+    (void)orb_octree_rule_from_env(P);
+    P.oct_team_force = force_team;
+    for (int l = 0; l < nlevels; l++) team_of_level[l] = orb_octree_team(P, l, batch);
+    OctGroup og[ORB_OCT_MAX_GROUPS];
+    const int ng = orb_octree_plan(P, batch, og);
+    for (int g = 0; g < ng; g++) {
+        long long *o = groups + 6 * g;
+        o[0] = og[g].team; o[1] = og[g].nlv; o[2] = og[g].nc; o[3] = (long long)orb_octree_lds_bytes(og[g].nc);
+        o[4] = (long long)og[g].lvls; o[5] = (long long)og[g].nlv * batch;
+    }
+    return ng;
 }
 
 extern "C" int orbhip_extractor_set_profiling(orbhip_extractor *e, int enable)
@@ -846,7 +897,28 @@
     STAGE_MARK(ORBHIP_STAGE_BLUR);
     if (!fork) orb_launch_blur(P, s, 8);
     STAGE_MARK(ORBHIP_STAGE_OCTREE);
-    orb_launch_octree(P, s);
+    {
+        OctGroup og[ORB_OCT_MAX_GROUPS];
+        const int ng = orb_octree_plan(P, batch, og);
+        const bool ofork = fork && ng > 1;
+        if (ofork && !(e->oct_aux_ok && e->ev_oct_fork)) {
+            if (e->oct_aux_ok) { g_last_error = "the octree streams could not be created earlier"; return ORBHIP_E_HIP; }
+            e->oct_aux_ok = true;
+            for (int i = 0; i < ORB_OCT_MAX_GROUPS - 1; i++) {
+                HIP_TRY(hipStreamCreateWithFlags(&e->oct_aux[i], hipStreamNonBlocking));
+                HIP_TRY(hipEventCreateWithFlags(&e->ev_oct_join[i], hipEventDisableTiming));
+            }
+            HIP_TRY(hipEventCreateWithFlags(&e->ev_oct_fork, hipEventDisableTiming));
+        }
+        if (ofork) HIP_TRY(hipEventRecord(e->ev_oct_fork, s));
+        orb_launch_octree(P, og[0], s);
+        for (int g = 1; g < ng; g++) {
+            hipStream_t so = ofork ? e->oct_aux[g - 1] : s;
+            if (ofork) HIP_TRY(hipStreamWaitEvent(so, e->ev_oct_fork, 0));
+            orb_launch_octree(P, og[g], so);
+            if (ofork) { HIP_TRY(hipEventRecord(e->ev_oct_join[g - 1], so)); HIP_TRY(hipStreamWaitEvent(s, e->ev_oct_join[g - 1], 0)); }
+        }
+    }
     STAGE_MARK(ORBHIP_STAGE_DESC);
     if (fork) HIP_TRY(hipStreamWaitEvent(s, e->ev_join, 0));
     orb_launch_orient_desc(P, s);
diff --git a/orb-slam3-mac_amd/python/orbhip.py b/orb-slam3-mac_amd/python/orbhip.py
--- a/orb-slam3-mac_amd/python/orbhip.py
+++ b/orb-slam3-mac_amd/python/orbhip.py
@@ -64,6 +64,13 @@
 lib.orbhip_extractor_blur_kernel.restype = ci
 lib.orbhip_extractor_resize_band_rows.argtypes = [vp, ci]
 lib.orbhip_extractor_resize_band_rows.restype = ci
+lib.orbhip_extractor_octree_team.argtypes = [vp, ci, ci]
+lib.orbhip_extractor_octree_team.restype = ci
+lib.orbhip_extractor_octree_caps.argtypes = [vp, ci, C.POINTER(ci), C.POINTER(ci)]
+lib.orbhip_octree_team_slots.argtypes = [ci]
+lib.orbhip_octree_team_slots.restype = ci
+lib.orbhip_octree_plan_query.argtypes = [ci, vp, vp, ci, ci, vp, vp]
+lib.orbhip_octree_plan_query.restype = ci
 lib.orbhip_prev_matched_init_device.argtypes = [vp, vp, sz, ci, ci, vp]
 lib.orbhip_search_by_projection_device.argtypes = [vp, vp, vp, vp, ci, vp, vp, vp, vp, ci, sz, ci, cf, cf, cf, cf, ci, ci, vp, vp]
 lib.orbhip_search_local_map_device.argtypes = [vp, vp, vp, vp, ci, vp, vp, vp, vp, ci, sz, ci, cf, cf, cf, cf, ci, cf, vp, vp]
@@ -145,6 +152,14 @@
 
     def resize_band_rows(self, level):
         return lib.orbhip_extractor_resize_band_rows(self.h, int(level))
+
+    def octree_caps(self, level):
+        a, b = ci(), ci()
+        _chk(lib.orbhip_extractor_octree_caps(self.h, int(level), C.byref(a), C.byref(b)), "octree_caps")
+        return a.value, b.value
+
+    def octree_team(self, level, batch):
+        return lib.orbhip_extractor_octree_team(self.h, int(level), int(batch))
 
     def set_graph_mode(self, on):
         _chk(lib.orbhip_extractor_set_graph_mode(self.h, 1 if on else 0), "orbhip_extractor_set_graph_mode")
@@ -222,6 +237,19 @@
         _chk(lib.orbhip_extractor_get_level_keypoints(self.h, frame, level, out.ctypes.data, cap, C.byref(n)),
              "get_level_keypoints")
         return out[:n.value].copy()
+
+
+def octree_plan(node_cap, key_cap, batch, force_team=0):
+    n = len(node_cap)
+    nc, kc = np.asarray(node_cap, np.int32), np.asarray(key_cap, np.int32)
+    team = np.zeros(n, np.int32)
+    groups = np.zeros(18, np.int64)
+    ng = lib.orbhip_octree_plan_query(n, nc.ctypes.data, kc.ctypes.data, int(batch), int(force_team), team.ctypes.data,
+                                      groups.ctypes.data)
+    if ng < 0:
+        raise OrbHipError(ng, "orbhip_octree_plan_query")
+    keys = ("team", "nlevels", "node_cap", "lds_bytes", "levels", "grid")
+    return team.tolist(), [dict(zip(keys, (int(v) for v in groups[6 * g:6 * g + 6]))) for g in range(ng)]
 
 
 def match_bf2nn_device(ctx, d_descA, d_nA, strideA, d_descB, d_nB, strideB, pairs, max_n, ratio, d_idx2, d_dist2,
```

Result: no change. 314,700 frames/s (-0.2%).
